# courtois-neuromod/phantom_vlb

Measured on AMD Instinct MI355X. Metric: clips/sec fine-tune VideoLLaMA2-7B+LoRA->2k-voxel head, 1/2/4/8 MI355X, higher is better.
Workload: dtype bf16; 1 GPU; configs[2]: VideoLLaMA2-7B + LoRA r=16 + 2k-voxel head, bf16; clips_per_gpu=3, global_batch=3, seq_len=2048, frames=12, num_target=2048, weights=random-init, comm=none

## Files before the change

### include/vlb.h

```cpp
#ifndef VLB_H
#define VLB_H

#include <stdint.h>

#ifdef __cplusplus
extern "C" {
#endif
#if defined(__GNUC__) || defined(__clang__)
#pragma GCC visibility push(default)
#endif

#define VLB_OK 0
#define VLB_ERR_INVALID (-1)
#define VLB_ERR_LAUNCH (-2)

#define VLB_ABI_VERSION 2

#define VLB_ACT_NONE 0
#define VLB_ACT_QUICK_GELU 1
#define VLB_ACT_GELU 2
#define VLB_ACT_SILU 3
#define VLB_ACT_SWIGLU_PAIR 4
#define VLB_ACT_SWIGLU_BWD 5

int vlb_abi_version(void);
const char* vlb_last_error(void);

int vlb_gemm_bf16(const void* A, int lda, const void* W, int ldw, void* C, int ldc, int M, int N, int K,
                  const void* bias, const void* residual, int ldr, int act, const void* A2, int lda2,
                  const void* W2, int ldw2, int K2, void* stream);

int vlb_gemm_bf16_ws(const void* A, int lda, const void* W, int ldw, void* C, int ldc, int M, int N, int K,
                     const void* bias, const void* residual, int ldr, int act, const void* A2, int lda2,
                     const void* W2, int ldw2, int K2, void* ws, int64_t ws_bytes, void* stream);
int vlb_gemm_swiglu_save(const void* A, int lda, const void* W_il, int ldw, void* H, int ldh, void* GU, int ldgu, int M, int N,
                         int K, const void* A2, int lda2, const void* W2_il, int ldw2, int K2, void* ws, int64_t ws_bytes,
                         void* stream);
int64_t vlb_gemm_workspace_bytes(void);
int vlb_gemm_plan(int M, int N, int K, int K2, int with_workspace);

int vlb_gemm_bf16_masked_pair(const void* A, int lda, const void* W, int ldw, void* C, int ldc, int M, int N, int K,
                              const void* A2, int lda2, const void* W2, int ldw2, float drop_p, uint32_t seed,
                              void* stream);

int vlb_gemm_bf16_masked_pair_ws(const void* A, int lda, const void* W, int ldw, void* C, int ldc, int M, int N, int K,
                                 const void* A2, int lda2, const void* W2, int ldw2, float drop_p, uint32_t seed,
                                 void* ws, int64_t ws_bytes, void* stream);

int vlb_gemm_masked_pair_swiglu_bwd(const void* dY, int lddy, const void* Wt, int ldw, const void* gu, int ldgu, void* dgu,
                                    int lddgu, int M, int ff, int K, const void* U, int ldu, const void* At, int ldat,
                                    float drop_p, uint32_t seed, void* ws, int64_t ws_bytes, void* stream);

int vlb_gemm_kernel_choice(int M, int N, int K, int K2);

int vlb_transpose_bf16(const void* in, void* out, int R, int C, void* stream);

int vlb_attention_fwd(const void* q, int ldq, const void* k, int ldk, const void* v, int ldv, void* out, int ldo,
                      float* lse, const uint8_t* key_mask, int B, int S, int Hq, int Hkv, int D, int causal,
                      float scale, const int* cu_rows, void* stream);

int vlb_attention_bwd(const void* q, int ldq, const void* k, int ldk, const void* v, int ldv, const void* out,
                      int ldo, const void* dout, int lddo, const float* lse, const uint8_t* key_mask, void* dq,
                      int lddq, void* dk, int lddk, void* dv, int lddv, float* delta, float* dq_acc, int B, int S,
                      int Hq, int Hkv, int D, int causal, float scale, const int* cu_rows, int total_rows,
                      void* stream);

int vlb_rmsnorm_fwd(const void* x, const void* w, void* y, int rows, int dim, float eps, void* stream);
int vlb_rmsnorm_bwd(const void* x, const void* w, const void* dy, const void* dx_in, void* dx, int rows, int dim,
                    float eps, void* stream);
int vlb_layernorm_fwd(const void* x, const void* w, const void* b, const void* residual, void* y, int rows, int dim,
                      float eps, int act, void* stream);

int vlb_rope_inplace(void* x, int ld, const float* cos_t, const float* sin_t, int rows, int S, int heads, int D,
                     int sign, const int* pos, void* stream);
int vlb_swiglu_fwd(const void* gu, void* out, int rows, int ff, void* stream);
int vlb_swiglu_bwd(const void* gu, const void* dout, void* dgu, int rows, int ff, void* stream);
int vlb_add_bf16(const void* a, const void* b, void* y, int64_t n, void* stream);

int vlb_patchify(const float* vision, void* patches, int N, int H, int W, int P, int Kpad, void* stream);
int vlb_vit_assemble(const void* patch_emb, const void* cls, const void* pos, void* tokens, int N, int G, int D,
                     void* stream);
int vlb_drop_cls(const void* tokens, void* out, int N, int G, int D, void* stream);

int vlb_dwconv3x3(const void* x, const void* w, void* y, int N, int H, int W, int C, void* stream);
int vlb_se_pool(const void* x, void* pooled, int N, int HW, int C, void* stream);
int vlb_se_scale(const void* x, const void* gate, void* y, int N, int HW, int C, void* stream);
int vlb_im2col3d_k2s2p1(const void* x, void* cols, int B, int T, int H, int W, int C, void* stream);

int vlb_splice_embed(const int64_t* ids, const void* embed_w, const void* video_tokens, void* embeds,
                     uint8_t* key_mask, int* err_flag, int B, int L, int Nv, int D, int64_t video_id, int vocab,
                     const int* cu_rows, int* row_pos, void* stream);
int vlb_weight_mask(const int64_t* padvals, const double* vis_w, const double* lang_w, float* wmask, int B, int F,
                    int Lw, int tokens_per_frame, int S, int round_bf16, void* stream);

int vlb_head_partial_rows(int S);
int64_t vlb_head_ws_floats(int B, int S, int E, int V);
int vlb_head_fwd(const void* hidden, const float* wmask, const void* ln1_w, const void* ln1_b, const void* ln2_w,
                 const void* ln2_b, const void* ridge_w, const void* ridge_b, const float* y, const float* keep_scale,
                 float* ws, float* stats, float* pooled_raw, float* sumw, float* zhat, float* ln2_rstd, void* z,
                 float* pred, float* loss_terms, int B, int S, int E, int V, float eps, float l2_lambda, const int* cu_rows,
                 void* stream);
int vlb_head_bwd(const void* hidden, const float* wmask, const void* ln1_w, const void* ln2_w, const void* ridge_w,
                 const float* y, const float* keep_scale, const float* stats, const float* pooled_raw,
                 const float* sumw, const float* zhat, const float* ln2_rstd, const void* z, const float* pred,
                 float* d_ridge_w, float* d_ridge_b, float* d_ln2_w, float* d_ln2_b, float* d_ln1_w, float* d_ln1_b,
                 float* ws, float* dz_ws, float* dpooled_ws, void* dhidden, int B, int S, int E, int V, float eps,
                 float l2_lambda, float loss_scale, float l2_scale, const int* cu_rows, int total_rows, void* stream);

int vlb_feature_cache_store(const float* pooled_raw, const float* sumw, const int32_t* rows, float* cache_pooled,
                            float* cache_sumw, int B, int E, int n_rows, void* stream);
int vlb_head_fwd_cached(const float* cache_pooled, const float* cache_sumw, const int32_t* rows, const void* ln1_w,
                        const void* ln1_b, const void* ln2_w, const void* ln2_b, const void* ridge_w, const void* ridge_b,
                        const float* y, const float* keep_scale, float* ws, float* pooled_raw, float* sumw, float* zhat,
                        float* ln2_rstd, void* z, float* pred, float* loss_terms, int B, int E, int V, int n_rows, float eps,
                        float l2_lambda, void* stream);
int vlb_head_bwd_cached(const void* ln1_w, const void* ln2_w, const void* ridge_w, const float* y, const float* keep_scale,
                        const float* pooled_raw, const float* sumw, const float* zhat, const float* ln2_rstd, const void* z,
                        const float* pred, float* d_ridge_w, float* d_ridge_b, float* d_ln2_w, float* d_ln2_b, float* d_ln1_w,
                        float* d_ln1_b, float* ws, float* dz_ws, float* dpooled_ws, int B, int E, int V, float eps,
                        float l2_lambda, float loss_scale, float l2_scale, void* stream);

int vlb_lora_down(const void* x, int ldx, const void* A, void* t, int ldt, int M, int K, int R, float scale,
                  float drop_p, const uint32_t* seeds_host, void* stream);
int vlb_lora_dx_masked(const void* u, int ldu, const void* At, int ldat, void* dx, int lddx, int M, int K, int R, float drop_p,
                       const uint32_t* seeds_host, void* stream);
int64_t vlb_wgrad_u_ws_floats(int M, int K);
int vlb_wgrad_skinny_u(const void* G, int ldg, const void* X, int ldx, float* dW, float* ws, int M, int K, float alpha,
                       float beta, const void* Bt, float u_scale, void* u, int ldu, float* u_ws, void* stream);
int vlb_wgrad_skinny_u_multi(const void* G, int ldg, const void* X, int ldx, int M, int nproj, const int* cols, float* const* dW,
                             const void* const* Bt, float* ws, float alpha, float beta, float u_scale, void* u, int ldu,
                             float* u_ws, void* stream);
int vlb_transpose16_scatter(const void* jobs, int n_jobs, void* stream);
int vlb_wgrad_splits(int M);
int vlb_wgrad_skinny(const void* G, int ldg, const void* X, int ldx, float* dW, float* ws, int M, int N, int K,
                     float alpha, float beta, float drop_p, const uint32_t* seeds_host, void* stream);

int vlb_sumsq_ws_floats(void);
int vlb_grad_sumsq(const float* g, int64_t n, float* sumsq, float* ws, void* stream);
int vlb_adamw_step(float* master, void* param_bf16, const float* grad, float* m, float* v, int64_t n, float lr,
                   float beta1, float beta2, float eps, float weight_decay, int step, const float* sumsq,
                   float max_norm, void* stream);
int vlb_grad_accum(float* acc, const float* g, int64_t n, int first, float* sumsq, float* ws, void* stream);
int vlb_grad_accum_bf16(float* acc, const void* g_bf16, int64_t n, int first, float* sumsq, float* ws, void* stream);

int vlb_transpose_pad(const void* in, int ld_in, void* out, int ld_out, int R, int C, int Rpad, void* stream);
int64_t vlb_norm_bwd_ws_floats(int rows, int dim);
int64_t vlb_colsum_ws_floats(int rows, int dim);
int vlb_rmsnorm_bwd_dw(const void* x, const void* dy, void* dw_bf16, float* ws, int rows, int dim, float eps, void* stream);
// ... 65 lines not shown
```

### phantom_vlb_amd/_lib.py

```python
from __future__ import annotations

import ctypes
import os
from ctypes import c_char_p, c_double, c_float, c_int, c_int64, c_void_p

import torch

_HERE = os.path.dirname(os.path.abspath(__file__))
LIB_PATH = os.environ.get("VLB_LIB") or os.path.join(_HERE, "libvlb.so")
IS_PRODUCT_LIB = os.path.abspath(LIB_PATH) == os.path.join(_HERE, "libvlb.so")

P, I, F, L = c_void_p, c_int, c_float, c_int64

SIGNATURES = {
    "vlb_abi_version": [],
    "vlb_last_error": [],
    "vlb_gemm_bf16": [P, I, P, I, P, I, I, I, I, P, P, I, I, P, I, P, I, I, P],
    "vlb_gemm_bf16_ws": [P, I, P, I, P, I, I, I, I, P, P, I, I, P, I, P, I, I, P, L, P],
    "vlb_gemm_swiglu_save": [P, I, P, I, P, I, P, I, I, I, I, P, I, P, I, I, P, L, P],
    "vlb_gemm_workspace_bytes": [],
    "vlb_gemm_plan": [I, I, I, I, I],
    "vlb_gemm_kernel_choice": [I, I, I, I],
    "vlb_transpose_bf16": [P, P, I, I, P],
    "vlb_attention_fwd": [P, I, P, I, P, I, P, I, P, P, I, I, I, I, I, I, F, P, P],
    "vlb_attention_bwd": [P, I, P, I, P, I, P, I, P, I, P, P, P, I, P, I, P, I, P, P, I, I, I, I, I, I, F, P, I, P],
    "vlb_rmsnorm_fwd": [P, P, P, I, I, F, P],
    "vlb_rmsnorm_bwd": [P, P, P, P, P, I, I, F, P],
    "vlb_layernorm_fwd": [P, P, P, P, P, I, I, F, I, P],
    "vlb_rope_inplace": [P, I, P, P, I, I, I, I, I, P, P],
    "vlb_swiglu_fwd": [P, P, I, I, P],
    "vlb_swiglu_bwd": [P, P, P, I, I, P],
    "vlb_add_bf16": [P, P, P, L, P],
    "vlb_patchify": [P, P, I, I, I, I, I, P],
    "vlb_vit_assemble": [P, P, P, P, I, I, I, P],
    "vlb_drop_cls": [P, P, I, I, I, P],
    "vlb_dwconv3x3": [P, P, P, I, I, I, I, P],
    "vlb_se_pool": [P, P, I, I, I, P],
    "vlb_se_scale": [P, P, P, I, I, I, P],
    "vlb_im2col3d_k2s2p1": [P, P, I, I, I, I, I, P],
    "vlb_splice_embed": [P, P, P, P, P, P, I, I, I, I, L, I, P, P, P],
    "vlb_weight_mask": [P, P, P, P, I, I, I, I, I, I, P],
    "vlb_head_partial_rows": [I],
    "vlb_head_ws_floats": [I, I, I, I],
    "vlb_head_fwd": [P] * 19 + [I, I, I, I, F, F, P, P],
    "vlb_head_bwd": [P] * 24 + [I, I, I, I, F, F, F, F, P, I, P],
    "vlb_feature_cache_store": [P] * 5 + [I, I, I, P],
    "vlb_head_fwd_cached": [P] * 19 + [I, I, I, I, F, F, P],
    "vlb_head_bwd_cached": [P] * 20 + [I, I, I, F, F, F, F, P],
    "vlb_gemm_bf16_masked_pair": [P, I, P, I, P, I, I, I, I, P, I, P, I, F, ctypes.c_uint32, P],
    "vlb_gemm_masked_pair_swiglu_bwd": [P, I, P, I, P, I, P, I, I, I, I, P, I, P, I, F, ctypes.c_uint32, P, L, P],
    "vlb_gemm_bf16_masked_pair_ws": [P, I, P, I, P, I, I, I, I, P, I, P, I, F, ctypes.c_uint32, P, L, P],
    "vlb_wgrad_u_ws_floats": [I, I],
    "vlb_wgrad_skinny_u": [P, I, P, I, P, P, I, I, F, F, P, F, P, I, P, P],
    "vlb_wgrad_skinny_u_multi": [P, I, P, I, I, I, P, P, P, P, F, F, F, P, I, P, P],
    "vlb_transpose16_scatter": [P, I, P],
    "vlb_wgrad_splits": [I],
    "vlb_wgrad_skinny": [P, I, P, I, P, P, I, I, I, F, F, F, P, P],
    "vlb_lora_down": [P, I, P, P, I, I, I, I, F, F, P, P],
    "vlb_lora_dx_masked": [P, I, P, I, P, I, I, I, I, F, P, P],
    "vlb_sumsq_ws_floats": [],
    "vlb_grad_sumsq": [P, L, P, P, P],
    "vlb_adamw_step": [P, P, P, P, P, L, F, F, F, F, F, I, P, F, P],
    "vlb_grad_accum": [P, P, L, I, P, P, P],
    "vlb_grad_accum_bf16": [P, P, L, I, P, P, P],
    "vlb_dropout_keep_scale": [P, L, F, ctypes.c_uint32, P],
    "vlb_transpose_pad": [P, I, P, I, I, I, I, P],
    "vlb_norm_bwd_ws_floats": [I, I],
    "vlb_colsum_ws_floats": [I, I],
    "vlb_rmsnorm_bwd_dw": [P, P, P, P, I, I, F, P],
    "vlb_rmsnorm_bwd_full_ws_floats": [I, I],
    "vlb_rmsnorm_bwd_full": [P, P, P, P, P, P, P, I, I, F, P],
    "vlb_layernorm_bwd": [P, P, P, P, P, P, P, P, P, P, I, I, F, I, P],
    "vlb_act_fwd": [P, P, L, I, P],
    "vlb_act_bwd": [P, P, P, L, I, P],
    "vlb_colsum": [P, I, P, P, I, I, P],
    "vlb_embed_grad": [P, I, P, P, P, I, P, I, P],
    "vlb_grad_sumsq_bf16": [P, L, P, P, P],
    "vlb_adamw_step_g16": [P, P, P, P, P, L, F, F, F, F, F, I, P, F, P],
    "vlb_dwconv3x3_bwd_w_ws_floats": [I, I, I],
    "vlb_dwconv3x3_bwd_w": [P, P, P, P, I, I, I, I, P],
    "vlb_se_bwd_gate": [P, P, P, P, I, I, I, P],
    "vlb_se_bwd_x": [P, P, P, P, I, I, I, P],
    "vlb_col2im3d_k2s2p1": [P, P, I, I, I, I, I, P],
    "vlb_quantize_mxfp8": [P, I, P, I, P, I, I, I, P],
    "vlb_transpose_quantize_mxfp8": [P, I, P, I, P, I, I, I, I, P],
    "vlb_quantize_dual_mxfp8": [P, I, P, I, P, I, P, I, P, I, I, I, I, P],
    "vlb_rmsnorm_fwd_mxfp8": [P, P, P, P, I, P, I, I, I, F, P],
    "vlb_swiglu_fwd_mxfp8": [P, P, P, I, P, I, I, I, P],
    "vlb_gemm_mxfp8": [P, I, P, I, P, I, P, I, P, I, I, I, I, P, I, P],
    "vlb_comm_unique_id": [P],
    "vlb_comm_init": [I, I, P, ctypes.POINTER(c_void_p)],
    "vlb_comm_destroy": [P],
    "vlb_comm_loopback_stage_bytes": [I],
    "vlb_comm_init_loopback": [I, P, L, ctypes.POINTER(c_void_p)],
    "vlb_comm_rank": [P],
    "vlb_comm_world": [P],
    "vlb_allgather_direct": [P, P, P, L, P],
    "vlb_reducescatter_stage_floats": [L, I],
    "vlb_reducescatter_direct": [P, P, P, L, P, P],
    "vlb_reducescatter_direct_bf16": [P, P, P, L, P, P],
    "vlb_reduce_slices": [P, P, L, I, I, P],
    "vlb_profile_marker": [P],
    "vlb_hrf_pool_ws_floats": [I, I],
    "vlb_hrf_pool": [P, I, P, P, P, I, I, I, P],
    "vlb_ridge_ws_floats": [I],
    "vlb_ridge_fwd": [P, P, P, P, P, P, I, I, I, F, P],
    "vlb_allreduce_scalar": [P, P, I, P],
    "vlb_cast_f32_to_bf16": [P, P, L, P],
# ... 36 lines not shown
```

### phantom_vlb_amd/csrc/attention.hip

```cpp
#include "common.hpp"

namespace {

constexpr int KV = 64;
constexpr int QW = 32;
constexpr int NW = 4;
constexpr int QB = QW * NW;
constexpr float NEG = -1e30f;

__device__ __forceinline__ void glds16(const void* g, void* l) {
  __builtin_amdgcn_global_load_lds((const void __attribute__((address_space(1)))*)g,
                                   (void __attribute__((address_space(3)))*)l, 16, 0, 0);
}

typedef short s16x4 __attribute__((ext_vector_type(4)));

__device__ __forceinline__ s16x4 tr_read_asm(const char* lds_ptr) {
  s16x4 v;
  const unsigned a = (unsigned)(uintptr_t)(const char __attribute__((address_space(3)))*)lds_ptr;
  asm volatile("ds_read_b64_tr_b16 %0, %1" : "=v"(v) : "v"(a));
  return v;
}
__device__ __forceinline__ void lds_wait_all() {
  asm volatile("s_waitcnt lgkmcnt(0)" ::: "memory");
// ... 182 lines not shown
          const int roff = (32 * s + 16 * s2) * ROWB;
#pragma unroll
          for (int dt = 0; dt < DT; ++dt) {
            const s16x4 lo = __builtin_amdgcn_ds_read_tr16_b64_v4i16(
                (s16x4 __attribute__((address_space(3)))*)(vb + v_rd[dt] + roff));
            const s16x4 hi = __builtin_amdgcn_ds_read_tr16_b64_v4i16(
                (s16x4 __attribute__((address_space(3)))*)(vb + v_rd[dt] + roff + 8 * ROWB));
            ot[dt] = __builtin_amdgcn_mfma_f32_32x32x16_bf16(join8(lo, hi), pf, ot[dt], 0, 0, 0);
          }
        }
    }
    asm volatile("s_waitcnt vmcnt(0)" ::: "memory");
    __syncthreads();
  }

  const float l_tot = l_run + __shfl_xor(l_run, 32, 64);
  const float inv = l_tot > 0.f ? 1.f / l_tot : 0.f;
  const int qrow = q0 + ql;
  if (qrow < Sb) {
    bf16* op = p.o + (row0 + qrow) * p.ldo + hq * D;
#pragma unroll
    for (int dt = 0; dt < DT; ++dt)
#pragma unroll
      for (int g = 0; g < 4; ++g) {
        bf16x4 o;
#pragma unroll
        for (int e = 0; e < 4; ++e) o[e] = (bf16)(ot[dt][4 * g + e] * inv);
        *reinterpret_cast<bf16x4*>(op + 32 * dt + 8 * g + 4 * h) = o;
      }
    if (p.lse && h == 0)
      p.lse[((int64_t)b * p.Hq + hq) * p.S + qrow] = l_tot > 0.f ? m_run * p.scale + logf(l_tot) : -INFINITY;
  }
}

template <int D, bool CAUSAL>
int launch_fwd(const AttnArgs& a, hipStream_t s) {
  constexpr int LDS = 2 * 2 * KV * D * 2;
  static const hipError_t attr = hipFuncSetAttribute(reinterpret_cast<const void*>(&attn_fwd_kernel<D, CAUSAL>),
                                                     hipFuncAttributeMaxDynamicSharedMemorySize, LDS);
  if (attr != hipSuccess) { vlb_set_error("attention: LDS reservation failed: %s", hipGetErrorString(attr)); return VLB_ERR_LAUNCH; }
  dim3 grid(((a.S + QB - 1) / QB) * a.Hq * a.B);
  hipLaunchKernelGGL((attn_fwd_kernel<D, CAUSAL>), grid, dim3(256), LDS, s, a);
  VLB_LAUNCH_CHECK();
  return VLB_OK;
}
}

extern "C" int vlb_attention_fwd(const void* q, int ldq, const void* k, int ldk, const void* v, int ldv, void* out,
                                 int ldo, float* lse, const uint8_t* key_mask, int B, int S, int Hq, int Hkv, int D,
                                 int causal, float scale, const int* cu_rows, void* stream) {
  VLB_REQUIRE(q && k && v && out, "attention_fwd: null operand");
  VLB_REQUIRE(D == 64 || D == 128, "attention_fwd: head dim %d not in {64,128}", D);
  VLB_REQUIRE(B > 0 && S > 0 && Hq > 0 && Hkv > 0 && Hq % Hkv == 0, "attention_fwd: bad shape B=%d S=%d Hq=%d Hkv=%d", B, S, Hq, Hkv);
  VLB_REQUIRE(ldq % 8 == 0 && ldk % 8 == 0 && ldv % 8 == 0 && ldo % 4 == 0, "attention_fwd: strides must keep 16-byte alignment");
  VLB_REQUIRE((((uintptr_t)q | (uintptr_t)k | (uintptr_t)v) % 16 == 0) && ((uintptr_t)out % 8 == 0), "attention_fwd: misaligned pointer");
  AttnArgs a{(const bf16*)q, (const bf16*)k, (const bf16*)v, (bf16*)out, lse, key_mask, cu_rows, ldq, ldk, ldv, ldo, B, S, Hq, Hkv, scale};
  hipStream_t s = as_stream(stream);
  if (D == 128) return causal ? launch_fwd<128, true>(a, s) : launch_fwd<128, false>(a, s);
  return causal ? launch_fwd<64, true>(a, s) : launch_fwd<64, false>(a, s);
}

namespace {

constexpr int BK_KEYS = 128;
constexpr int BQ = 32;

#ifdef VLB_TOOLS
int g_attn_ablate = 0;
#else
constexpr int g_attn_ablate = 0;
#endif
struct AttnBwdArgs {
  const bf16* q; const bf16* k; const bf16* v; const bf16* dout;
  const float* lse; const float* delta; const uint8_t* mask; const int* cu;
  bf16* dk; bf16* dv; float* dq_acc;
  int ldq, ldk, ldv, lddo, lddk, lddv;
  int B, S, Hq, Hkv;
  float scale;
  int ablate;
};

__device__ __forceinline__ int sw2(int r) { return ((r & 3) << 2) | ((r >> 2) & 3); }

__global__ __launch_bounds__(256) void attn_delta_kernel(const bf16* __restrict__ o, int ldo, const bf16* __restrict__ d_o,
                                                         int lddo, float* __restrict__ delta, int S, int Hq, int B,
                                                         const int* __restrict__ cu, int64_t total) {
  const int64_t gid = (int64_t)blockIdx.x * 16 + (threadIdx.x >> 4);
  const int c = threadIdx.x & 15;
  float s = 0.f;
  if (gid < total) {
    const int h = gid % Hq; const int64_t tok = gid / Hq;
    const bf16x8 a = *reinterpret_cast<const bf16x8*>(o + tok * ldo + h * 128 + c * 8);
    const bf16x8 b = *reinterpret_cast<const bf16x8*>(d_o + tok * lddo + h * 128 + c * 8);
#pragma unroll
    for (int i = 0; i < 8; ++i) s += (float)a[i] * (float)b[i];
  }
#pragma unroll
  for (int off = 8; off > 0; off >>= 1) s += __shfl_xor(s, off, 64);
  if (gid < total && c == 0) {
    const int h = gid % Hq; const int64_t tok = gid / Hq;
    int64_t b = tok / S; int sidx = tok % S;
    if (cu) {
      int bb = 0;
      while (bb + 1 < B && tok >= cu[bb + 1]) ++bb;
      b = bb; sidx = (int)(tok - cu[bb]);
    }
    delta[(b * Hq + h) * S + sidx] = s;
  }
}

template <bool CAUSAL>
__global__ __launch_bounds__(256, 2) void attn_bwd_dkdv_kernel(AttnBwdArgs p, bf16* __restrict__ part) {
  constexpr int D = 128, ROWB = 256;
  constexpr int V_OFF = 0;
  constexpr int QT_BYTES = BQ * ROWB;
  constexpr int Q_OFF = BK_KEYS * ROWB;
  constexpr int L_OFF = Q_OFF + 4 * QT_BYTES;
  extern __shared__ __attribute__((aligned(16))) char smem[];

  const int tid = threadIdx.x, lane = tid & 63;
  const int w4 = __builtin_amdgcn_readfirstlane(tid >> 6);
  const int per_kb = p.Hq * p.B;
  const int kb = blockIdx.x / per_kb, hq = xcd_head((blockIdx.x % per_kb) % p.Hq, p.Hq), b = (blockIdx.x % per_kb) / p.Hq;
  const int gsz = p.Hq / p.Hkv;
  const int hkv = hq / gsz;
  const int k0 = kb * BK_KEYS;
  const int Sb = p.cu ? p.cu[b + 1] - p.cu[b] : p.S;
  const int64_t row0 = p.cu ? p.cu[b] : (int64_t)b * p.S;
  if (k0 >= Sb) return;
  const int ql = lane & 31, h = lane >> 5;
  const int g1 = (lane >> 4) & 1, li = lane & 15, tq = li >> 2, tp = li & 3;
  const int sr = lane >> 4, sp = lane & 15;

  const int krow = w4 * 32 + ql;
  const int key = k0 + krow;
  bf16x8 kf[8];
  {
    const bf16* kp = p.k + (row0 + min(key, Sb - 1)) * p.ldk + hkv * D + 8 * h;
#pragma unroll
    for (int ks = 0; ks < 8; ++ks) kf[ks] = *reinterpret_cast<const bf16x8*>(kp + 16 * ks);
  }
  const bf16* vbase = p.v + row0 * p.ldv + hkv * D;
#pragma unroll
  for (int i = 0; i < 8; ++i) {
    const int piece = 4 * i + w4, r = piece * 4 + sr;
    glds16(vbase + (int64_t)min(k0 + r, Sb - 1) * p.ldv + (sp ^ sw2(r)) * 8, smem + V_OFF + piece * 1024);
  }
  const int nqb = (Sb + BQ - 1) / BQ;
  const int qb0 = CAUSAL ? (k0 / BQ) : 0;
  const int total = nqb - qb0;
  const bf16* qbase = p.q + row0 * p.ldq + hq * D;
  const bf16* dobase = p.dout + row0 * p.lddo + hq * D;
  const float* lsebase = p.lse + ((int64_t)b * p.Hq + hq) * p.S;
  const float* delbase = p.delta + ((int64_t)b * p.Hq + hq) * p.S;

  auto stage_q = [&](int buf, int item) {
    const int qb = qb0 + item;
    char* qt = smem + Q_OFF + buf * 2 * QT_BYTES;
#pragma unroll
    for (int i = 0; i < 2; ++i) {
      const int piece = 4 * i + w4, r = piece * 4 + sr;
      const int qr = min(qb * BQ + r, Sb - 1);
      glds16(qbase + (int64_t)qr * p.ldq + (sp ^ sw2(r)) * 8, qt + piece * 1024);
      glds16(dobase + (int64_t)qr * p.lddo + (sp ^ sw2(r)) * 8, qt + QT_BYTES + piece * 1024);
    }
    if (w4 == 0) {
      const int qr = min(qb * BQ + (lane & 31), Sb - 1);
      const float* src = (lane < 32 ? lsebase : delbase) + qr;
      __builtin_amdgcn_global_load_lds((const void __attribute__((address_space(1)))*)src,
                                       (void __attribute__((address_space(3)))*)(smem + L_OFF + buf * 256), 4, 0, 0);
    }
  };

  f32x16 dkt[4], dvt[4];
#pragma unroll
  for (int i = 0; i < 4; ++i)
#pragma unroll
    for (int r = 0; r < 16; ++r) { dkt[i][r] = 0.f; dvt[i][r] = 0.f; }
// ... 38 lines not shown
        pacc = __builtin_amdgcn_mfma_f32_32x32x16_bf16(dof, vf, pacc, 0, 0, 0);
      }
      bf16x8 pb[2], dsb[2];
#pragma unroll
      for (int g = 0; g < 4; ++g) {
        const f32x4 l4 = *reinterpret_cast<const f32x4*>(ls + 8 * g + 4 * h);
        const f32x4 d4 = *reinterpret_cast<const f32x4*>(ls + 32 + 8 * g + 4 * h);
#pragma unroll
        for (int e = 0; e < 4; ++e) {
          const int r = 4 * g + e;
          const int qrow = q0 + 8 * g + 4 * h + e;
          bool ok = key_ok && qrow < Sb;
          if (CAUSAL) ok = ok && (key <= qrow);
          const float pv = ok ? __builtin_amdgcn_exp2f(sacc[r] * c2 - l4[e] * 1.44269504088896341f) : 0.f;
          const float ds = pv * (pacc[r] - d4[e]) * p.scale;
          pb[r >> 3][r & 7] = (bf16)pv;
          dsb[r >> 3][r & 7] = (bf16)ds;
        }
      }
#pragma unroll
      for (int s = 0; s < 2; ++s) {
        s16x4 ra[4][2];
#pragma unroll
        for (int dt = 0; dt < 4; ++dt)
#pragma unroll
          for (int e = 0; e < 2; ++e) ra[dt][e] = tr_read_asm(dot + qt_rd[dt][e] + 16 * s * ROWB);
        lds_wait_all();
#pragma unroll
        for (int dt = 0; dt < 4; ++dt)
          dvt[dt] = __builtin_amdgcn_mfma_f32_32x32x16_bf16(join8(ra[dt][0], ra[dt][1]), pb[s], dvt[dt], 0, 0, 0);
#pragma unroll
        for (int dt = 0; dt < 4; ++dt)
#pragma unroll
          for (int e = 0; e < 2; ++e) ra[dt][e] = tr_read_asm(qt + qt_rd[dt][e] + 16 * s * ROWB);
        lds_wait_all();
#pragma unroll
        for (int dt = 0; dt < 4; ++dt)
          dkt[dt] = __builtin_amdgcn_mfma_f32_32x32x16_bf16(join8(ra[dt][0], ra[dt][1]), dsb[s], dkt[dt], 0, 0, 0);
      }
    }
    asm volatile("s_waitcnt vmcnt(0)" ::: "memory");
    asm volatile("s_waitcnt lgkmcnt(0)" ::: "memory");
    __builtin_amdgcn_s_barrier();
  }

  if (key < Sb) {
    bf16* dkp = gsz == 1 ? p.dk + (row0 + key) * p.lddk + hkv * D : part + ((row0 + key) * p.Hq + hq) * (2 * D);
    bf16* dvp = gsz == 1 ? p.dv + (row0 + key) * p.lddv + hkv * D : dkp + D;
#pragma unroll
    for (int dt = 0; dt < 4; ++dt)
#pragma unroll
      for (int g = 0; g < 4; ++g) {
        bf16x4 a, c;
#pragma unroll
        for (int e = 0; e < 4; ++e) { a[e] = (bf16)dkt[dt][4 * g + e]; c[e] = (bf16)dvt[dt][4 * g + e]; }
        *reinterpret_cast<bf16x4*>(dkp + 32 * dt + 8 * g + 4 * h) = a;
        *reinterpret_cast<bf16x4*>(dvp + 32 * dt + 8 * g + 4 * h) = c;
      }
  }
}

__global__ __launch_bounds__(256) void attn_dkdv_reduce_kernel(const bf16* __restrict__ part, bf16* __restrict__ dk, int lddk,
                                                               bf16* __restrict__ dv, int lddv, int Hq, int Hkv, int64_t total) {
  const int64_t i = blockIdx.x * (int64_t)blockDim.x + threadIdx.x;
  if (i >= total) return;
  const int c = i & 15, which = (i >> 4) & 1;
  const int hkv = (int)((i >> 5) % Hkv);
  const int64_t row = (i >> 5) / Hkv;
  const int gsz = Hq / Hkv;
  float acc[8] = {0.f, 0.f, 0.f, 0.f, 0.f, 0.f, 0.f, 0.f};
  const bf16* src = part + (row * Hq + (int64_t)hkv * gsz) * 256 + which * 128 + c * 8;
  for (int j = 0; j < gsz; ++j) {
    const bf16x8 v = *reinterpret_cast<const bf16x8*>(src + (int64_t)j * 256);
#pragma unroll
    for (int e = 0; e < 8; ++e) acc[e] += (float)v[e];
  }
  bf16x8 o;
#pragma unroll
  for (int e = 0; e < 8; ++e) o[e] = (bf16)acc[e];
  bf16* dst = which ? dv + row * lddv : dk + row * lddk;
  *reinterpret_cast<bf16x8*>(dst + hkv * 128 + c * 8) = o;
}

struct AttnDqArgs {
  const bf16* q; const bf16* k; const bf16* v; const bf16* dout;
  const float* lse; const float* delta; const uint8_t* mask; const int* cu;
  bf16* dq;
  int ldq, ldk, ldv, lddo, lddq;
  int B, S, Hq, Hkv;
  float scale;
};

template <bool CAUSAL>
__global__ __launch_bounds__(256, 2) void attn_bwd_dq_kernel(AttnDqArgs p) {
  constexpr int D = 128, ROWB = 256, TILE = KV * ROWB, KS = 8, DT = 4;
  extern __shared__ __attribute__((aligned(16))) char smem[];

  const int tid = threadIdx.x, lane = tid & 63;
  const int wave = __builtin_amdgcn_readfirstlane(tid >> 6);
  const int nqb = (p.S + QB - 1) / QB;
  const int per_qb = p.Hq * p.B, slot = blockIdx.x / per_qb;
  const int qb = CAUSAL ? (nqb - 1 - slot) : slot;
  const int hq = xcd_head((blockIdx.x % per_qb) % p.Hq, p.Hq), b = (blockIdx.x % per_qb) / p.Hq;
  const int hkv = hq / (p.Hq / p.Hkv);
  const int Sb = p.cu ? p.cu[b + 1] - p.cu[b] : p.S;
  const int64_t row0 = p.cu ? p.cu[b] : (int64_t)b * p.S;
  if (qb * QB >= Sb) return;
  const int q0 = qb * QB + wave * QW;
  const int ql = lane & 31, h = lane >> 5;
  const int qrow = q0 + ql;
  const int qr = min(qrow, Sb - 1);

  bf16x8 qf[KS], dof[KS];
  {
    const bf16* qp = p.q + (row0 + qr) * p.ldq + hq * D + 8 * h;
    const bf16* dp = p.dout + (row0 + qr) * p.lddo + hq * D + 8 * h;
#pragma unroll
    for (int ks = 0; ks < KS; ++ks) {
      qf[ks] = *reinterpret_cast<const bf16x8*>(qp + 16 * ks);
      dof[ks] = *reinterpret_cast<const bf16x8*>(dp + 16 * ks);
    }
  }
  const float lse_q = p.lse[((int64_t)b * p.Hq + hq) * p.S + qr];
  const float delta_q = p.delta[((int64_t)b * p.Hq + hq) * p.S + qr];
  const float c2 = p.scale * 1.44269504088896341f;
  const float lse2 = (lse_q > -1e37f) ? lse_q * 1.44269504088896341f : 1e37f;

  f32x16 dqt[DT];
#pragma unroll
  for (int i = 0; i < DT; ++i)
#pragma unroll
    for (int r = 0; r < 16; ++r) dqt[i][r] = 0.f;

  const int q_hi = min(qb * QB + QB, Sb) - 1;
  const int ntiles = CAUSAL ? (q_hi / KV + 1) : (Sb + KV - 1) / KV;
  const bf16* kbase = p.k + row0 * p.ldk + hkv * D;
  const bf16* vbase = p.v + row0 * p.ldv + hkv * D;

  const int sr = lane >> 4, sp = lane & 15;
  auto stage = [&](int buf, int t) {
    char* kb = smem + buf * 2 * TILE; char* vb = kb + TILE;
#pragma unroll
    for (int i = 0; i < 4; ++i) {
      const int r = (4 * i + wave) * 4 + sr;
      const int key = min(t * KV + r, Sb - 1);
      glds16(kbase + (int64_t)key * p.ldk + (sp ^ sw2(r)) * 8, kb + (4 * i + wave) * 1024);
      glds16(vbase + (int64_t)key * p.ldv + (sp ^ sw2(r)) * 8, vb + (4 * i + wave) * 1024);
    }
  };
  stage(0, 0);
  asm volatile("s_waitcnt vmcnt(0)" ::: "memory");
  __syncthreads();

  const int g1 = (lane >> 4) & 1, li = lane & 15, tq = li >> 2, tp = li & 3;
  int row_rd[KS];
#pragma unroll
  for (int ks = 0; ks < KS; ++ks) row_rd[ks] = ql * ROWB + (((2 * ks + h) ^ sw2(ql)) << 4);
  int tr_rd[DT][2];
#pragma unroll
  for (int dt = 0; dt < DT; ++dt)
#pragma unroll
    for (int e = 0; e < 2; ++e) {
      const int r = 4 * h + tq + 8 * e;
      tr_rd[dt][e] = r * ROWB + (((4 * dt + 2 * g1 + (tp >> 1)) ^ sw2(r)) << 4) + (tp & 1) * 8;
    }

  for (int t = 0; t < ntiles; ++t) {
    const int cur = t & 1;
    if (t + 1 < ntiles) stage(cur ^ 1, t + 1);
    const char* kb = smem + cur * 2 * TILE; const char* vb = kb + TILE;
    const int key0 = t * KV;
    const bool active = !CAUSAL || (key0 <= q0 + QW - 1);
    if (active) {
      f32x16 st[2], dp[2];
#pragma unroll
      for (int s = 0; s < 2; ++s)
#pragma unroll
        for (int r = 0; r < 16; ++r) { st[s][r] = 0.f; dp[s][r] = 0.f; }
#pragma unroll
      for (int ks = 0; ks < KS; ++ks) {
#pragma unroll
        for (int s = 0; s < 2; ++s) {
          const bf16x8 kf = *reinterpret_cast<const bf16x8*>(kb + row_rd[ks] + 32 * s * ROWB);
          st[s] = __builtin_amdgcn_mfma_f32_32x32x16_bf16(kf, qf[ks], st[s], 0, 0, 0);
          const bf16x8 vf = *reinterpret_cast<const bf16x8*>(vb + row_rd[ks] + 32 * s * ROWB);
          dp[s] = __builtin_amdgcn_mfma_f32_32x32x16_bf16(vf, dof[ks], dp[s], 0, 0, 0);
        }
      }
      unsigned long long kvalid;
      {
        const int key = key0 + lane;
        bool ok = key < Sb;
        if (ok && p.mask) ok = p.mask[row0 + key] != 0;
        kvalid = __ballot(ok);
      }
      const bool diag = CAUSAL && (key0 + KV - 1 > q0);
      const bool partial = diag || (kvalid != ~0ull);
      if (partial) {
        const unsigned lo = (unsigned)(kvalid >> (4 * h)), hi = (unsigned)(kvalid >> (32 + 4 * h));
#pragma unroll
        for (int s = 0; s < 2; ++s) {
          const unsigned word = s ? hi : lo;
#pragma unroll
          for (int r = 0; r < 16; ++r) {
            const int kb2 = (r & 3) + 8 * (r >> 2);
            bool ok = (word >> kb2) & 1u;
            if (CAUSAL) ok = ok && (key0 + 32 * s + 4 * h + kb2 <= qrow);
            st[s][r] = ok ? st[s][r] : NEG;
          }
        }
        asm volatile("" ::: "memory");
      }
#pragma unroll
      for (int s = 0; s < 2; ++s)
#pragma unroll
        for (int r = 0; r < 16; ++r) {
          const float pv = __builtin_amdgcn_exp2f(st[s][r] * c2 - lse2);
          st[s][r] = pv * (dp[s][r] - delta_q) * p.scale;
        }
#pragma unroll
      for (int s = 0; s < 2; ++s)
#pragma unroll
        for (int s2 = 0; s2 < 2; ++s2) {
          bf16x8 df;
#pragma unroll
          for (int j = 0; j < 8; ++j) df[j] = (bf16)st[s][8 * s2 + j];
          const int roff = (32 * s + 16 * s2) * ROWB;
#pragma unroll
          for (int dt = 0; dt < DT; ++dt) {
            const s16x4 lo = __builtin_amdgcn_ds_read_tr16_b64_v4i16(
                (s16x4 __attribute__((address_space(3)))*)(kb + tr_rd[dt][0] + roff));
            const s16x4 hi = __builtin_amdgcn_ds_read_tr16_b64_v4i16(
                (s16x4 __attribute__((address_space(3)))*)(kb + tr_rd[dt][1] + roff));
            dqt[dt] = __builtin_amdgcn_mfma_f32_32x32x16_bf16(join8(lo, hi), df, dqt[dt], 0, 0, 0);
          }
        }
    }
    asm volatile("s_waitcnt vmcnt(0)" ::: "memory");
    __syncthreads();
  }

  if (qrow < Sb) {
    bf16* op = p.dq + (row0 + qrow) * p.lddq + hq * D;
#pragma unroll
    for (int dt = 0; dt < DT; ++dt)
#pragma unroll
      for (int g = 0; g < 4; ++g) {
        bf16x4 o;
#pragma unroll
        for (int e = 0; e < 4; ++e) o[e] = (bf16)dqt[dt][4 * g + e];
        *reinterpret_cast<bf16x4*>(op + 32 * dt + 8 * g + 4 * h) = o;
      }
  }
}

}

extern "C" int vlb_attention_bwd(const void* q, int ldq, const void* k, int ldk, const void* v, int ldv, const void* out,
                                 int ldo, const void* dout, int lddo, const float* lse, const uint8_t* key_mask, void* dq,
                                 int lddq, void* dk, int lddk, void* dv, int lddv, float* delta, float* dq_acc, int B,
                                 int S, int Hq, int Hkv, int D, int causal, float scale, const int* cu_rows, int total_rows,
                                 void* stream) {
  VLB_REQUIRE(q && k && v && out && dout && lse && dq && dk && dv && delta, "attention_bwd: null operand");
  VLB_REQUIRE(dq_acc || Hq == Hkv, "attention_bwd: the [rows, Hq, D] fp32-sized workspace is required");
  VLB_REQUIRE(D == 128, "attention_bwd: head dim %d unsupported (only 128: the decoder)", D);
  VLB_REQUIRE(B > 0 && S > 0 && Hq > 0 && Hkv > 0 && Hq % Hkv == 0, "attention_bwd: bad shape");
  VLB_REQUIRE(ldq % 8 == 0 && ldk % 8 == 0 && ldv % 8 == 0 && ldo % 8 == 0 && lddo % 8 == 0 && lddq % 8 == 0 &&
                  lddk % 4 == 0 && lddv % 4 == 0, "attention_bwd: strides must keep vector alignment");
  VLB_REQUIRE(((((uintptr_t)q | (uintptr_t)k | (uintptr_t)v | (uintptr_t)out | (uintptr_t)dout) % 16) == 0) &&
                  ((uintptr_t)dq % 8 == 0), "attention_bwd: misaligned pointer");
  hipStream_t st = as_stream(stream);
  const int64_t rows = cu_rows ? (int64_t)total_rows : (int64_t)B * S;
  VLB_REQUIRE(rows > 0 && rows <= (int64_t)B * S, "attention_bwd: total_rows=%d out of range", total_rows);
  const int64_t th = rows * Hq;
  hipLaunchKernelGGL(attn_delta_kernel, dim3((unsigned)((th + 15) / 16)), dim3(256), 0, st, (const bf16*)out, ldo,
                     (const bf16*)dout, lddo, delta, S, Hq, B, cu_rows, th);
  VLB_LAUNCH_CHECK();
  AttnBwdArgs a{(const bf16*)q, (const bf16*)k, (const bf16*)v, (const bf16*)dout, lse, delta, key_mask, cu_rows,
                (bf16*)dk, (bf16*)dv, dq_acc, ldq, ldk, ldv, lddo, lddk, lddv, B, S, Hq, Hkv, scale, g_attn_ablate};
  dim3 grid((S + BK_KEYS - 1) / BK_KEYS, Hkv, B);
  {
    const int gsz = Hq / Hkv;
    VLB_REQUIRE(gsz == 1 || dq_acc, "attention_bwd: the workspace (fp32 [rows, Hq, D]) is required for grouped-query heads");
    VLB_REQUIRE(lddk % 8 == 0 && lddv % 8 == 0 && (((uintptr_t)dk | (uintptr_t)dv) % 16) == 0, "attention_bwd: dk/dv rows must be 16-byte aligned");
    constexpr int LDS_KV = BK_KEYS * 256 + 4 * BQ * 256 + 512;
    static const hipError_t k1 = hipFuncSetAttribute(reinterpret_cast<const void*>(&attn_bwd_dkdv_kernel<true>), hipFuncAttributeMaxDynamicSharedMemorySize, LDS_KV);
    static const hipError_t k2 = hipFuncSetAttribute(reinterpret_cast<const void*>(&attn_bwd_dkdv_kernel<false>), hipFuncAttributeMaxDynamicSharedMemorySize, LDS_KV);
    if (k1 != hipSuccess || k2 != hipSuccess) { vlb_set_error("attention_bwd: LDS reservation failed (dk/dv)"); return VLB_ERR_LAUNCH; }
    bf16* part = reinterpret_cast<bf16*>(dq_acc);
    dim3 gridh(grid.x * Hq * B);
    if (causal) hipLaunchKernelGGL(attn_bwd_dkdv_kernel<true>, gridh, dim3(256), LDS_KV, st, a, part);
    else hipLaunchKernelGGL(attn_bwd_dkdv_kernel<false>, gridh, dim3(256), LDS_KV, st, a, part);
    VLB_LAUNCH_CHECK();
    if (gsz > 1) {
      const int64_t tot = rows * Hkv * 32;
      hipLaunchKernelGGL(attn_dkdv_reduce_kernel, dim3((unsigned)((tot + 255) / 256)), dim3(256), 0, st, part, (bf16*)dk, lddk,
                         (bf16*)dv, lddv, Hq, Hkv, tot);
      VLB_LAUNCH_CHECK();
    }
  }
  AttnDqArgs d{(const bf16*)q, (const bf16*)k, (const bf16*)v, (const bf16*)dout, lse, delta, key_mask, cu_rows,
               (bf16*)dq, ldq, ldk, ldv, lddo, lddq, B, S, Hq, Hkv, scale};
  constexpr int LDS_DQ = 2 * 2 * KV * 256;
  static const hipError_t q1 = hipFuncSetAttribute(reinterpret_cast<const void*>(&attn_bwd_dq_kernel<true>), hipFuncAttributeMaxDynamicSharedMemorySize, LDS_DQ);
  static const hipError_t q2 = hipFuncSetAttribute(reinterpret_cast<const void*>(&attn_bwd_dq_kernel<false>), hipFuncAttributeMaxDynamicSharedMemorySize, LDS_DQ);
  if (q1 != hipSuccess || q2 != hipSuccess) { vlb_set_error("attention_bwd: LDS reservation failed (dq)"); return VLB_ERR_LAUNCH; }
  dim3 gq(((S + QB - 1) / QB) * Hq * B);
  if (causal) hipLaunchKernelGGL(attn_bwd_dq_kernel<true>, gq, dim3(256), LDS_DQ, st, d);
  else hipLaunchKernelGGL(attn_bwd_dq_kernel<false>, gq, dim3(256), LDS_DQ, st, d);
  VLB_LAUNCH_CHECK();
  return VLB_OK;
}

#ifdef VLB_TOOLS
extern "C" void vlb_attn_set_ablation(int bits) { g_attn_ablate = bits & 3; }
#endif
```

### phantom_vlb_amd/csrc/common.hpp

```cpp
#pragma once
#include <hip/hip_runtime.h>
#include <stdint.h>
#include <stdio.h>
#include <string.h>

#include "../../include/vlb.h"

typedef __bf16 bf16;
typedef __bf16 bf16x2 __attribute__((ext_vector_type(2)));
typedef __bf16 bf16x4 __attribute__((ext_vector_type(4)));
typedef __bf16 bf16x8 __attribute__((ext_vector_type(8)));
typedef float f32x2 __attribute__((ext_vector_type(2)));
typedef float f32x4 __attribute__((ext_vector_type(4)));
typedef float f32x16 __attribute__((ext_vector_type(16)));
typedef unsigned int u32x2 __attribute__((ext_vector_type(2)));
typedef unsigned int u32x4 __attribute__((ext_vector_type(4)));

#define VLB_WAVE 64

void vlb_set_error(const char* fmt, ...);

#define VLB_REQUIRE(cond, ...)                 \
  do {                                         \
    if (!(cond)) {                             \
      vlb_set_error(__VA_ARGS__);              \
      return VLB_ERR_INVALID;                  \
    }                                          \
  } while (0)

#define VLB_LAUNCH_CHECK()                                                   \
  do {                                                                       \
    hipError_t e__ = hipGetLastError();                                      \
    if (e__ != hipSuccess) {                                                 \
      vlb_set_error("%s:%d launch failed: %s", __FILE__, __LINE__,           \
                    hipGetErrorString(e__));                                 \
      return VLB_ERR_LAUNCH;                                                 \
    }                                                                        \
  } while (0)

static inline hipStream_t as_stream(void* s) {
  (void)hipGetLastError();
  return reinterpret_cast<hipStream_t>(s);
}

__device__ __forceinline__ float bf2f(bf16 x) { return (float)x; }
__device__ __forceinline__ bf16 f2bf(float x) { return (bf16)x; }

__device__ __forceinline__ float wave_sum(float v) {
#pragma unroll
  for (int o = 32; o > 0; o >>= 1) v += __shfl_xor(v, o, 64);
  return v;
}
__device__ __forceinline__ float wave_max(float v) {
#pragma unroll
  for (int o = 32; o > 0; o >>= 1) v = fmaxf(v, __shfl_xor(v, o, 64));
  return v;
}

__device__ __forceinline__ float block_sum(float v, float* red) {
  v = wave_sum(v);
  const int w = threadIdx.x >> 6, nw = blockDim.x >> 6;
  __syncthreads();
  if ((threadIdx.x & 63) == 0) red[w] = v;
  __syncthreads();
  float t = 0.f;
  for (int i = 0; i < nw; ++i) t += red[i];
  return t;
}

__device__ __forceinline__ float sigmoid_f(float x) { return __builtin_amdgcn_rcpf(1.f + __expf(-x)); }
__device__ __forceinline__ float silu_f(float x) { return x * sigmoid_f(x); }
__device__ __forceinline__ float quick_gelu_f(float x) { return x * sigmoid_f(1.702f * x); }
__device__ __forceinline__ float gelu_erf_f(float x) { return 0.5f * x * (1.f + erff(x * 0.70710678118654752f)); }

__device__ __forceinline__ int mx_shared_exp(float amax) {
  int E = -127;
  if (amax > 0.f) {
    int e; const float f = frexpf(amax / 448.f, &e);
    E = (f == 0.5f) ? e - 1 : e;
    E = max(-127, min(127, E));
  }
  return E;
}
__device__ __forceinline__ uint32_t mx_pack4(float a, float b, float c, float d, float inv) {
  int pk = 0;
  pk = __builtin_amdgcn_cvt_pk_fp8_f32(a * inv, b * inv, pk, false);
  pk = __builtin_amdgcn_cvt_pk_fp8_f32(c * inv, d * inv, pk, true);
  return (uint32_t)pk;
}
__device__ __forceinline__ void mx_quantize_lane8(const float (&v)[8], uint8_t* qrow, uint8_t* srow, int c, int lane) {
  float amax = 0.f;
#pragma unroll
  for (int i = 0; i < 8; ++i) amax = fmaxf(amax, fabsf(v[i]));
  amax = fmaxf(amax, __shfl_xor(amax, 1, 64));
  amax = fmaxf(amax, __shfl_xor(amax, 2, 64));
  const int E = mx_shared_exp(amax);
  const float inv = exp2f((float)-E);
  typedef unsigned u32x2_ __attribute__((ext_vector_type(2)));
  *reinterpret_cast<u32x2_*>(qrow + c) = u32x2_{mx_pack4(v[0], v[1], v[2], v[3], inv), mx_pack4(v[4], v[5], v[6], v[7], inv)};
  if ((lane & 3) == 0) srow[c >> 5] = (uint8_t)(E + 127);
}
__device__ __forceinline__ void load_pair16(const bf16* row, int n, int fq, bf16x4& a, bf16x4& b) {
  typedef unsigned u32x2 __attribute__((ext_vector_type(2)));
  typedef unsigned u32x4 __attribute__((ext_vector_type(4)));
  const u32x4 l = *reinterpret_cast<const u32x4*>(row + n + ((fq & 1) ? 12 : 0));
  const auto r0 = __builtin_amdgcn_permlane16_swap(l[0], l[2], false, false);
  const auto r1 = __builtin_amdgcn_permlane16_swap(l[1], l[3], false, false);
  a = __builtin_bit_cast(bf16x4, u32x2{r0[0], r1[0]});
  b = __builtin_bit_cast(bf16x4, u32x2{r0[1], r1[1]});
}
__device__ __forceinline__ void store_pair16(bf16* row, int n, bf16x4 a, bf16x4 b, int fq) {
  typedef unsigned u32x2 __attribute__((ext_vector_type(2)));
  typedef unsigned u32x4 __attribute__((ext_vector_type(4)));
  u32x2 ua = __builtin_bit_cast(u32x2, a), ub = __builtin_bit_cast(u32x2, b);
  const auto r0 = __builtin_amdgcn_permlane16_swap(ua[0], ub[0], false, false);
  const auto r1 = __builtin_amdgcn_permlane16_swap(ua[1], ub[1], false, false);
  const u32x4 o = {r0[0], r1[0], r0[1], r1[1]};
  *reinterpret_cast<u32x4*>(row + n + ((fq & 1) ? 12 : 0)) = o;
}
```

### phantom_vlb_amd/csrc/gemm.hip

```cpp
#include <type_traits>

#include "common.hpp"

namespace {

constexpr int BK = 64;
constexpr int ROW_BYTES = BK * 2;

struct GemmArgs {
  const bf16* A;  const bf16* W;  bf16* C;
  const bf16* A2; const bf16* W2;
  const bf16* bias; const bf16* residual;
  int M, N, K, K2;
  int lda, ldw, ldc, ldr, lda2, ldw2;
  int act;
  int tiles_m, tiles_n;
  int tile0;
  int split_n;
  int grid;
  uint32_t drop_thresh, drop_key; float drop_scale;
  float* ws; int k_splits, tail_tiles;
  int order;
  bf16* aux; int ldaux;
  int reserved;
  int wide;
};

__device__ __forceinline__ void tile_coords(const GemmArgs& p, int pid, int sub, int BM, int BN, int& m0, int& n0) {
  int tm, tn;
  if (p.order & 4) {
    const int sbt = 16 * p.tiles_m;
    const int sb = pid / sbt, c0 = sb * 16;
    const int wd = min(p.tiles_n - c0, 16);
    int w = pid - sb * sbt;
    const int rg = w / (4 * wd);
    const int gsz = min(p.tiles_m - 4 * rg, 4);
    w -= rg * 4 * wd;
    const int h = w / (gsz * 8);
    const int cw = min(wd - 8 * h, 8);
    w -= h * gsz * 8;
    tm = 4 * rg + w / cw;
    tn = c0 + 8 * h + w % cw;
  } else if (p.order & 1) {
    constexpr int GROUP_N = 8;
    const int band = GROUP_N * p.tiles_m;
    const int cb = pid / band, c0 = cb * GROUP_N;
    const int csz = min(p.tiles_n - c0, GROUP_N);
    const int w = pid - cb * band;
    tm = w / csz;
    tn = c0 + w % csz;
  } else {
    constexpr int GROUP_M = 4;
    const int band = GROUP_M * p.tiles_n;
    const int g0 = (pid / band) * GROUP_M;
    const int gsz = min(p.tiles_m - g0, GROUP_M);
    tm = g0 + (pid % band) % gsz;
    tn = (pid % band) / gsz;
  }
  m0 = tm * BM;
  n0 = (tn * p.split_n + sub) * BN;
}

__device__ __forceinline__ int xcd_remap_pid(int order) {
  const int nblk = gridDim.x, pid = blockIdx.x;
  const int x = pid & 7, j = pid >> 3;
  int base = 0, n = nblk, jj = j;
  if (order & 2) {
    const int T = nblk >> 8, t = j >> 5;
    if (t < T) return (t << 8) + (x << 5) + (j & 31);
    base = T << 8; n = nblk - base; jj = j - (T << 5);
  }
  const int q = n >> 3, r = n & 7;
  return base + (x < r ? x * (q + 1) : r * (q + 1) + (x - r) * q) + jj;
}

__device__ __forceinline__ int map_tile(const GemmArgs& p, int BM, int BN, int& m0, int& n0) {
  int pid = xcd_remap_pid(p.order);
  int sub = 0, ks = 0;
  if (p.split_n > 1) { sub = pid % p.split_n; pid /= p.split_n; }
  if (p.k_splits > 1) { ks = pid / p.tail_tiles; pid -= ks * p.tail_tiles; }
  tile_coords(p, pid + p.tile0, sub, BM, BN, m0, n0);
  return ks;
}

__device__ __forceinline__ float apply_act(float x, int act) {
  switch (act) {
    case VLB_ACT_QUICK_GELU: return quick_gelu_f(x);
    case VLB_ACT_GELU: return gelu_erf_f(x);
    case VLB_ACT_SILU: return silu_f(x);
    default: return x;
  }
}

__device__ __forceinline__ void store_swiglu4(const GemmArgs& p, const f32x4& g, const f32x4& u, int m, int n) {
  bf16x4 o;
#pragma unroll
  for (int e = 0; e < 4; ++e) o[e] = (bf16)(silu_f(g[e]) * u[e]);
  *reinterpret_cast<bf16x4*>(p.C + (int64_t)m * p.ldc + n) = o;
  if (p.aux) {
    bf16x4 gb, ub;
#pragma unroll
    for (int e = 0; e < 4; ++e) { gb[e] = (bf16)g[e]; ub[e] = (bf16)u[e]; }
    bf16* ap = p.aux + (int64_t)m * p.ldaux + n;
    *reinterpret_cast<bf16x4*>(ap) = gb;
    *reinterpret_cast<bf16x4*>(ap + (p.N >> 1)) = ub;
  }
}

// ... 492 lines not shown
        if (g >= 1 && (g * 4) % NT == 0 && g * 4 / NT - 1 <= MT - 2) af[g * 4 / NT - 1] = frag(sn, a_off[0], g * 4 / NT - 1);
        if (g == LAST_A) a7[0] = frag(sn, a_off[0], MT - 1);
      }
#pragma unroll
      for (int q = 0; q < 4; ++q) {
        const int t = g * 4 + q, i = t / NT, j = t % NT;
        mfma_tied(acc[i][j], wf[1][j], i == MT - 1 ? a7[1] : af[i]);
      }
      W4_FENCE();
    }
    __builtin_amdgcn_s_waitcnt(0xc07f);
    asm volatile("s_nop 15" ::: "memory");
    W4_FENCE();
  };
  using T_ = std::true_type; using F_ = std::false_type;
  int kt = 0;
  if constexpr (MASKED) {
    const bool later_range = SPLITK && ksplit != 0;
    const uint32_t m_thresh = later_range ? 0u : p.drop_thresh;
    const float m_scale = later_range ? 1.f : p.drop_scale;
    tile(0, T_{}, T_{});
    kt = 1;
    asm volatile("s_nop 15\n\ts_nop 15" ::: "memory");
#pragma unroll
    for (int i = 0; i < MT; ++i)
#pragma unroll
      for (int j = 0; j < NT; j += 4)
        asm volatile("" : "+a"(acc[i][j]), "+a"(acc[i][j + 1]), "+a"(acc[i][j + 2]), "+a"(acc[i][j + 3]));
    const int frm = lane & 15, fqm = lane >> 4;
    const uint32_t halfN = (uint32_t)(p.N >> 1);
#pragma unroll
    for (int i = 0; i < MT; ++i) {
      const uint32_t rb = (uint32_t)(m0 + wm * TM + i * 16 + frm) * halfN;
#pragma unroll
      for (int j = 0; j < NT; ++j) {
        const uint32_t pair0 = (uint32_t)(n0 + wn * TN + j * 16 + fqm * 4) >> 1;
        f32x4 v = acc[i][j];
#pragma unroll
        for (int q = 0; q < 2; ++q) {
          uint32_t h = (rb + pair0 + q) ^ p.drop_key;
          h ^= h >> 16; h *= 0x7feb352dU; h ^= h >> 15; h *= 0x846ca68bU; h ^= h >> 16;
          v[2 * q] = (h & 0xffffu) >= m_thresh ? v[2 * q] * m_scale : 0.f;
          v[2 * q + 1] = (h >> 16) >= m_thresh ? v[2 * q + 1] * m_scale : 0.f;
        }
        acc[i][j] = v;
        asm volatile("" : "+a"(acc[i][j]));
        W4_FENCE();
      }
    }
    asm volatile("s_nop 7" ::: "memory");
  }
  for (; kt + 2 < nk; ++kt) tile(kt, T_{}, T_{});
  if (kt + 1 < nk) { tile(kt, T_{}, F_{}); ++kt; }
  tile(kt, F_{}, F_{});
  asm volatile("s_nop 15\n\ts_nop 15" ::: "memory");
#pragma unroll
  for (int i = 0; i < MT; ++i)
#pragma unroll
    for (int j = 0; j < NT; j += 4)
      asm volatile("" : "+a"(acc[i][j]), "+a"(acc[i][j + 1]), "+a"(acc[i][j + 2]), "+a"(acc[i][j + 3]));
#undef W4_FENCE
#undef W4_BARRIER

  if constexpr (SPLITK) {
    float* wt = p.ws + ((int64_t)xcd_remap_pid(p.order) * 4 + wave) * (MT * NT * 256);
#pragma unroll
    for (int i = 0; i < MT; ++i)
#pragma unroll
      for (int j = 0; j < NT; ++j)
        *reinterpret_cast<f32x4*>(wt + ((i * NT + j) * 64 + lane) * 4) = acc[i][j];
    return;
  }
  if (p.act == VLB_ACT_SWIGLU_PAIR) {
#pragma unroll
    for (int i = 0; i < MT; ++i) {
      const int m = m0 + wm * TM + i * 16 + fr;
      if (m >= p.M) continue;
#pragma unroll
      for (int j = 0; j < NT; j += 4)
        store_swiglu8(p, acc[i][j], acc[i][j + 1], acc[i][j + 2], acc[i][j + 3], m, (n0 + wn * TN) / 2 + (j / 2) * 16 + fq * 4, fq);
    }
    return;
  }
#define W4_EPILOGUE(KIND)                                                                                              \
  _Pragma("unroll") for (int i = 0; i < MT; ++i) {                                                                      \
    const int m = m0 + wm * TM + i * 16 + fr;                                                                           \
    if (m >= p.M) continue;                                                                                             \
    _Pragma("unroll") for (int j = 0; j < NT; j += 2)                                                                   \
      w4_store_frag2<KIND>(p, acc[i][j], acc[i][j + 1], m, n0 + wn * TN + j * 16 + fq * 4, fq);                         \
  }
  const int kind = w4_epilogue_kind(p);
  if (kind == EPI_PLAIN) { W4_EPILOGUE(EPI_PLAIN) return; }
  if (kind == EPI_RESIDUAL) { W4_EPILOGUE(EPI_RESIDUAL) return; }
  if (kind == EPI_SWIGLU_BWD) { W4_EPILOGUE(EPI_SWIGLU_BWD) return; }
#define W4_EPILOGUE_ACT(ACT) W4_EPILOGUE(EPI_GENERIC + ACT)
  VLB_DISPATCH_ACT(p.act, W4_EPILOGUE_ACT);
#undef W4_EPILOGUE_ACT
#undef W4_EPILOGUE
}

template <int MT, int NT>
__global__ __launch_bounds__(256) void gemm_splitk_reduce_kernel(GemmArgs p) {
  constexpr int TM = 16 * MT, TN = 16 * NT, BM = 2 * TM, BN = 2 * TN;
  const int tl = blockIdx.x / MT, i = blockIdx.x % MT;
  int m0, n0;
  tile_coords(p, p.tile0 + tl, 0, BM, BN, m0, n0);
  const int lane = threadIdx.x & 63, wave = threadIdx.x >> 6;
  const int wm = wave >> 1, wn = wave & 1, fr = lane & 15, fq = lane >> 4;
  f32x4 v[NT];
#pragma unroll
  for (int j = 0; j < NT; ++j) v[j] = f32x4{0.f, 0.f, 0.f, 0.f};
  for (int s = 0; s < p.k_splits; ++s) {
    const float* wt = p.ws + ((int64_t)(s * p.tail_tiles + tl) * 4 + wave) * (MT * NT * 256);
#pragma unroll
    for (int j = 0; j < NT; ++j) v[j] += *reinterpret_cast<const f32x4*>(wt + ((i * NT + j) * 64 + lane) * 4);
  }
  const int m = m0 + wm * TM + i * 16 + fr;
  if (m >= p.M) return;
  if (p.act == VLB_ACT_SWIGLU_PAIR) {
#pragma unroll
    for (int j = 0; j < NT; j += 4) store_swiglu8(p, v[j], v[j + 1], v[j + 2], v[j + 3], m, (n0 + wn * TN) / 2 + (j / 2) * 16 + fq * 4, fq);
    return;
  }
  const int kind = w4_epilogue_kind(p);
#define W4_REDUCE_EPILOGUE(KIND) \
  _Pragma("unroll") for (int j = 0; j < NT; j += 2) w4_store_frag2<KIND>(p, v[j], v[j + 1], m, n0 + wn * TN + j * 16 + fq * 4, fq);
  if (kind == EPI_PLAIN) { W4_REDUCE_EPILOGUE(EPI_PLAIN) return; }
  if (kind == EPI_RESIDUAL) { W4_REDUCE_EPILOGUE(EPI_RESIDUAL) return; }
  if (kind == EPI_SWIGLU_BWD) { W4_REDUCE_EPILOGUE(EPI_SWIGLU_BWD) return; }
#define W4_REDUCE_EPILOGUE_ACT(ACT) W4_REDUCE_EPILOGUE(EPI_GENERIC + ACT)
  VLB_DISPATCH_ACT(p.act, W4_REDUCE_EPILOGUE_ACT);
#undef W4_REDUCE_EPILOGUE_ACT
#undef W4_REDUCE_EPILOGUE
}

template <int NT, int ABL, int MT = 8, bool MASKED = false, bool SPLITK = false>
int launch_w4(GemmArgs& a, hipStream_t s) {
  constexpr int LDS = 2 * (32 * MT + 32 * NT) * ROW_BYTES;
  static const hipError_t attr = hipFuncSetAttribute(reinterpret_cast<const void*>(&gemm_w4_kernel<NT, ABL, MT, MASKED, SPLITK>),
                                       hipFuncAttributeMaxDynamicSharedMemorySize, LDS);
  if (attr != hipSuccess) {
    vlb_set_error("gemm: cannot reserve %d bytes of LDS: %s", LDS, hipGetErrorString(attr));
    return VLB_ERR_LAUNCH;
  }
  hipLaunchKernelGGL((gemm_w4_kernel<NT, ABL, MT, MASKED, SPLITK>), dim3(a.grid), dim3(256), LDS, s, a);
  VLB_LAUNCH_CHECK();
  return VLB_OK;
}

template <int MT, bool MASKED = false>
int launch_w4_splitk(GemmArgs& a, hipStream_t s) {
  a.split_n = 1;
  a.grid = a.k_splits * a.tail_tiles;
  int rc = launch_w4<8, 0, MT, MASKED, true>(a, s);
  if (rc != VLB_OK) return rc;
  hipLaunchKernelGGL((gemm_splitk_reduce_kernel<MT, 8>), dim3(a.tail_tiles * MT), dim3(256), 0, s, a);
  VLB_LAUNCH_CHECK();
  return VLB_OK;
}

#ifdef VLB_TOOLS
#define VLB_TUNABLE
#else
#define VLB_TUNABLE constexpr
#endif
VLB_TUNABLE int g_variant = 3;
// ... 63 lines not shown
  return launch_pp<BM, BN, WM, WN, (BM + BN) / 64, 0, 0, 0>(a, s, LDS);
#else
  if constexpr (BM == 256 && BN == 256) {
    if (!fits32 && (g_variant == 2 || (g_variant >= 0x20 && g_variant < 0x30))) return launch_pp<BM, BN, WM, WN, (BM + BN) / 64, 0, 0, 0>(a, s, LDS);
    if (g_variant == 2) return launch_w4<8, 0>(a, s);
    if (g_variant == 3 || g_variant == 4 || g_variant == 5 || g_variant == 6) {
      if (fits32 && a.K + a.K2 >= 4096) return launch_w4<8, 0>(a, s);
      return launch_pp<BM, BN, WM, WN, (BM + BN) / 64, 0, 0, 0>(a, s, LDS);
    }
    if (g_variant == 0x21) return launch_w4<8, 1>(a, s);
    if (g_variant == 0x22) return launch_w4<8, 2>(a, s);
    if (g_variant == 0x24) return launch_w4<8, 4>(a, s);
    if (g_variant == 0x27) return launch_w4<8, 7>(a, s);
    if (g_variant == 0x28) return launch_w4<8, 8>(a, s);
    if (g_variant == 0x41) return launch_w4<8, 16>(a, s);
    if (g_variant == 0x42) return launch_w4<8, 32>(a, s);
    if (g_variant == 0x43) return launch_w4<8, 48>(a, s);
  } else {
    if constexpr (BM == 256 && BN == 128) {
      if ((g_variant == 2 || g_variant == 3 || g_variant == 5 || g_variant == 6) && fits32 && a.K + a.K2 >= 4096) return launch_w4<4, 0>(a, s);
    }
    if (g_variant == 2 || g_variant == 3 || g_variant == 4 || g_variant == 5 || g_variant == 6 || g_variant >= 0x20) return launch_pp<BM, BN, WM, WN, (BM + BN) / 64, 0, 0, 0>(a, s, LDS);
  }
  if (g_variant == 1) return launch_pp<BM, BN, WM, WN, (BM + BN) / 64, 0, 0, 0>(a, s, LDS);
  constexpr int T = (BM + BN) / 64;
  if constexpr (BM == 256 && BN == 256) {
    if (g_variant == 0x11) return launch_pp<BM, BN, WM, WN, T, 0, 0, 0, 1>(a, s, LDS);
    if (g_variant == 0x12) return launch_pp<BM, BN, WM, WN, T, 0, 0, 0, 2>(a, s, LDS);
    if (g_variant == 0x14) return launch_pp<BM, BN, WM, WN, T, 0, 0, 0, 4>(a, s, LDS);
    if (g_variant == 0x13) return launch_pp<BM, BN, WM, WN, T, 0, 0, 0, 3>(a, s, LDS);
    if (g_variant == 0x17) return launch_pp<BM, BN, WM, WN, T, 0, 0, 0, 7>(a, s, LDS);
    if (g_variant == 0x16) return launch_pp<BM, BN, WM, WN, T, 0, 0, 0, 6>(a, s, LDS);
  }
  if (g_variant >= 0x10) return launch_pp<BM, BN, WM, WN, T, 0, 0, 0>(a, s, LDS);
  vlb_set_error("gemm: unknown kernel variant %d", g_variant);
  return VLB_ERR_INVALID;
#endif
}

__global__ void transpose_kernel(const bf16* __restrict__ in, bf16* __restrict__ out, int R, int C) {
  __shared__ bf16 t[32][33];
  const int c0 = blockIdx.x * 32, r0 = blockIdx.y * 32;
  for (int i = threadIdx.y; i < 32; i += blockDim.y) {
    const int r = r0 + i, c = c0 + threadIdx.x;
    if (r < R && c < C) t[i][threadIdx.x] = in[(int64_t)r * C + c];
  }
  __syncthreads();
  for (int i = threadIdx.y; i < 32; i += blockDim.y) {
    const int c = c0 + i, r = r0 + threadIdx.x;
    if (r < R && c < C) out[(int64_t)c * R + r] = t[threadIdx.x][i];
  }
}

}

extern "C" int vlb_gemm_kernel_choice(int M, int N, int K, int K2) {
  if (K % BK != 0 || K2 % BK != 0 || K == 0 || M < 128) return 0;
  const int cus = 256;
  if (N % 256 == 0) {
    const int t256 = ((M + 255) / 256) * (N / 256);
    if (t256 < cus / 2) return 2;
    return 1;
  }
  if (N % 128 == 0) return 2;
  return 0;
}

extern "C" int vlb_gemm_plan(int M, int N, int K, int K2, int with_workspace) {
  if (N % 256 != 0 || K + K2 < 4096) return 0;
  TailPlan p256, p192;
  const bool use192 = plan_rows(M, N, K + K2, (with_workspace & 1) != 0, p256, p192, !(with_workspace & 2));
  const TailPlan& t = use192 ? p192 : p256;
  return (use192 ? 192 : 256) * 1000 + t.mode * 100 + t.splits;
}

extern "C" int64_t vlb_gemm_workspace_bytes(void) { return 256ll * 256 * 256 * 4; }

extern "C" int vlb_gemm_bf16(const void* A, int lda, const void* W, int ldw, void* C, int ldc, int M, int N, int K,
                             const void* bias, const void* residual, int ldr, int act, const void* A2, int lda2,
                             const void* W2, int ldw2, int K2, void* stream) {
  return vlb_gemm_bf16_ws(A, lda, W, ldw, C, ldc, M, N, K, bias, residual, ldr, act, A2, lda2, W2, ldw2, K2, nullptr, 0, stream);
}

static int gemm_impl(const void* A, int lda, const void* W, int ldw, void* C, int ldc, int M, int N, int K,
                     const void* bias, const void* residual, int ldr, int act, const void* A2, int lda2,
                     const void* W2, int ldw2, int K2, void* ws, int64_t ws_bytes, void* stream, void* aux, int ldaux);

extern "C" int vlb_gemm_bf16_ws(const void* A, int lda, const void* W, int ldw, void* C, int ldc, int M, int N, int K,
                                const void* bias, const void* residual, int ldr, int act, const void* A2, int lda2,
                                const void* W2, int ldw2, int K2, void* ws, int64_t ws_bytes, void* stream) {
  return gemm_impl(A, lda, W, ldw, C, ldc, M, N, K, bias, residual, ldr, act, A2, lda2, W2, ldw2, K2, ws, ws_bytes, stream, nullptr, 0);
}

extern "C" int vlb_gemm_swiglu_save(const void* A, int lda, const void* W_il, int ldw, void* H, int ldh, void* GU, int ldgu, int M, int N,
                                    int K, const void* A2, int lda2, const void* W2_il, int ldw2, int K2, void* ws, int64_t ws_bytes,
                                    void* stream) {
  VLB_REQUIRE(GU && ldgu >= N && ldgu % 4 == 0 && N % 8 == 0 && ((uintptr_t)GU % 8) == 0,
              "gemm_swiglu_save: [gate | up] rows must hold N columns, 8-byte aligned (N=%d ldgu=%d)", N, ldgu);
  return gemm_impl(A, lda, W_il, ldw, H, ldh, M, N, K, nullptr, nullptr, 0, VLB_ACT_SWIGLU_PAIR, A2, lda2, W2_il, ldw2, K2, ws, ws_bytes,
                   stream, GU, ldgu);
}

static int gemm_impl(const void* A, int lda, const void* W, int ldw, void* C, int ldc, int M, int N, int K,
                     const void* bias, const void* residual, int ldr, int act, const void* A2, int lda2,
                     const void* W2, int ldw2, int K2, void* ws, int64_t ws_bytes, void* stream, void* aux, int ldaux) {
  VLB_REQUIRE(A && W && C, "gemm: null operand");
  VLB_REQUIRE(!ws || ((uintptr_t)ws % 16) == 0, "gemm: workspace must be 16-byte aligned");
  const bool ws_ok = ws && ws_bytes >= vlb_gemm_workspace_bytes();
  VLB_REQUIRE(M > 0 && N > 0 && K > 0, "gemm: bad shape M=%d N=%d K=%d", M, N, K);
  VLB_REQUIRE(K % 8 == 0 && lda % 8 == 0 && ldw % 8 == 0, "gemm: K/lda/ldw must be multiples of 8 (K=%d lda=%d ldw=%d)", K, lda, ldw);
  VLB_REQUIRE(lda >= K && ldw >= K && (ldc >= N || (act == VLB_ACT_SWIGLU_PAIR && ldc >= N / 2)), "gemm: leading dimension smaller than row");
  if (K2 > 0) {
    VLB_REQUIRE(A2 && W2, "gemm: K2>0 needs A2 and W2");
    VLB_REQUIRE(K2 % 8 == 0 && lda2 % 8 == 0 && ldw2 % 8 == 0 && lda2 >= K2 && ldw2 >= K2, "gemm: bad second operand pair");
  } else {
    A2 = nullptr; W2 = nullptr; K2 = 0;
  }
  if (residual) VLB_REQUIRE(ldr >= N, "gemm: ldr < N");
  if (act == VLB_ACT_SWIGLU_PAIR) {
    VLB_REQUIRE(N % 32 == 0 && !bias && !residual && ldc >= N / 2, "gemm: SWIGLU_PAIR needs N %% 32 == 0, no bias/residual, ldc >= N/2");
  }
  GemmArgs a;
  a.A = (const bf16*)A; a.W = (const bf16*)W; a.C = (bf16*)C;
  a.A2 = (const bf16*)A2; a.W2 = (const bf16*)W2;
  a.bias = (const bf16*)bias; a.residual = (const bf16*)residual;
  a.M = M; a.N = N; a.K = K; a.K2 = K2;
  a.lda = lda; a.ldw = ldw; a.ldc = ldc; a.ldr = ldr; a.lda2 = lda2; a.ldw2 = ldw2;
  a.act = act; a.tiles_m = 0; a.tiles_n = 0; a.tile0 = 0; a.split_n = 1; a.grid = 0; a.drop_thresh = 0; a.drop_key = 0; a.drop_scale = 1.f;
  a.ws = nullptr; a.k_splits = 0; a.tail_tiles = 0; a.order = pick_order(M, N, K); a.aux = (bf16*)aux; a.ldaux = ldaux;
  a.wide = ((uintptr_t)C % 16) == 0 && ldc % 8 == 0 && (!aux || (((uintptr_t)aux % 16) == 0 && ldaux % 8 == 0 && (N / 2) % 8 == 0));
  hipStream_t s = as_stream(stream);
  const bool vec_ok = (ldc % 4 == 0) && (!residual || ldr % 4 == 0) && (!aux || (ldaux % 4 == 0 && (N / 2) % 4 == 0)) &&
                      (((uintptr_t)C | (uintptr_t)residual | (uintptr_t)bias | (uintptr_t)aux) % 8 == 0) &&
                      (((uintptr_t)A | (uintptr_t)W | (uintptr_t)A2 | (uintptr_t)W2) % 16 == 0);
  int choice = vec_ok ? vlb_gemm_kernel_choice(M, N, K, K2) : 0;
  if (choice != 0 && g_force_tile == 1 && N % 256 == 0) choice = 1;
  if (choice != 0 && g_force_tile == 2 && N % 128 == 0) choice = 2;
  if (choice == 1) {
    const int cus = 256, tn = N / 256, tm = (M + 255) / 256;
    const int tiles = tm * tn, rem = tiles % cus;
    {
      const bool fits32 = a.wide && (int64_t)M * lda < (1ll << 31) && (int64_t)N * ldw < (1ll << 31) &&
                          (int64_t)M * lda2 < (1ll << 31) && (int64_t)N * ldw2 < (1ll << 31);
#ifdef VLB_TOOLS
      const int abl192 = (g_variant >= 0x30 && g_variant < 0x40) ? (g_variant & 0xf) : 0;
      const bool w4 = (g_variant == 3 || g_variant == 5 || g_variant == 6 || (g_variant >= 0x30 && g_variant < 0x40)) && fits32 && K + K2 >= 4096;
#else
      const bool w4 = (g_variant == 3 || g_variant == 5) && fits32 && K + K2 >= 4096;
#endif
      const int tm192 = (M + 191) / 192, tiles192 = tm192 * tn;
      TailPlan p256, p192;
      bool use192 = plan_rows(M, N, K + K2, ws_ok && w4, p256, p192);
#ifdef VLB_TOOLS
      if (g_variant == 6) use192 = false;
#endif
      if (w4 && g_force_tile == 0 && tiles > cus && (g_variant == 5 || (g_variant >= 0x30 && g_variant < 0x40) || use192)) {
        GemmArgs hi = a;
        hi.tiles_m = tm192; hi.tiles_n = tn; hi.tile0 = 0; hi.split_n = 1;
        const int rem192 = tiles192 % cus;
        hi.grid = p192.mode ? tiles192 - rem192 : tiles192;
#ifdef VLB_TOOLS
        if (abl192 == 1) return launch_w4<8, 1, 6>(hi, s);
        if (abl192 == 2) return launch_w4<8, 2, 6>(hi, s);
        if (abl192 == 4) return launch_w4<8, 4, 6>(hi, s);
        if (abl192 == 8) return launch_w4<8, 8, 6>(hi, s);
        if (abl192 == 7) return launch_w4<8, 7, 6>(hi, s);
        if (abl192 == 9) return launch_w4<8, 16, 6>(hi, s);
        if (abl192 == 10) return launch_w4<8, 32, 6>(hi, s);
        if (abl192 == 11) return launch_w4<8, 48, 6>(hi, s);
#endif
        int rc = launch_w4<8, 0, 6>(hi, s);
        if (rc != VLB_OK || !p192.mode) return rc;
        GemmArgs lo = hi;
        lo.tile0 = tiles192 - rem192;
        if (p192.mode == 2) {
          lo.ws = (float*)ws; lo.k_splits = p192.splits; lo.tail_tiles = rem192;
          return launch_w4_splitk<6>(lo, s);
        }
        lo.split_n = 2; lo.grid = 2 * rem192;
        return launch_w4<4, 0, 6>(lo, s);
      }
      if (w4 && g_force_tile == 0 && p256.mode == 2) {
        GemmArgs hi = a;
        hi.tiles_m = tm; hi.tiles_n = tn; hi.tile0 = 0; hi.split_n = 1; hi.grid = tiles - rem;
        int rc = launch_w4<8, 0, 8>(hi, s);
        if (rc != VLB_OK) return rc;
        GemmArgs lo = hi;
        lo.tile0 = tiles - rem; lo.ws = (float*)ws; lo.k_splits = p256.splits; lo.tail_tiles = rem;
        return launch_w4_splitk<8>(lo, s);
      }
    }
    if (g_tail_split && tiles > cus && rem != 0 && rem <= cus * 5 / 8) {
      GemmArgs hi = a, lo = a;
      hi.tiles_m = lo.tiles_m = tm;
      hi.tiles_n = lo.tiles_n = tn;
      hi.tile0 = 0; hi.split_n = 1; hi.grid = tiles - rem;
      lo.tile0 = tiles - rem; lo.split_n = 2; lo.grid = 2 * rem;
      int rc = launch_tile<256, 256, 2, 4>(hi, s);
      if (rc != VLB_OK) return rc;
      return launch_tile<256, 128, 4, 2>(lo, s);
    }
    return launch_tile<256, 256, 2, 4>(a, s);
  }
  if (choice == 2) return launch_tile<256, 128, 4, 2>(a, s);
  dim3 grid((N + 63) / 64, (M + 63) / 64);
  hipLaunchKernelGGL(gemm_generic_kernel, grid, dim3(256), 0, s, a);
  VLB_LAUNCH_CHECK();
  return VLB_OK;
}

namespace {
inline uint32_t lowbias32_h(uint32_t x) {
  x ^= x >> 16; x *= 0x7feb352dU; x ^= x >> 15; x *= 0x846ca68bU; x ^= x >> 16;
  return x;
}
}

extern "C" int vlb_gemm_bf16_masked_pair(const void* A, int lda, const void* W, int ldw, void* C, int ldc, int M, int N, int K,
                                         const void* A2, int lda2, const void* W2, int ldw2, float drop_p, uint32_t seed,
                                         void* stream) {
  return vlb_gemm_bf16_masked_pair_ws(A, lda, W, ldw, C, ldc, M, N, K, A2, lda2, W2, ldw2, drop_p, seed, nullptr, 0, stream);
}

static int masked_pair_impl(const void* A, int lda, const void* W, int ldw, void* C, int ldc, int M, int N, int K,
                            const void* A2, int lda2, const void* W2, int ldw2, float drop_p, uint32_t seed,
                            void* ws, int64_t ws_bytes, void* stream, int act, const void* residual, int ldr);

extern "C" int vlb_gemm_bf16_masked_pair_ws(const void* A, int lda, const void* W, int ldw, void* C, int ldc, int M, int N, int K,
                                            const void* A2, int lda2, const void* W2, int ldw2, float drop_p, uint32_t seed,
                                            void* ws, int64_t ws_bytes, void* stream) {
  return masked_pair_impl(A, lda, W, ldw, C, ldc, M, N, K, A2, lda2, W2, ldw2, drop_p, seed, ws, ws_bytes, stream, VLB_ACT_NONE, nullptr, 0);
}

extern "C" int vlb_gemm_masked_pair_swiglu_bwd(const void* dY, int lddy, const void* Wt, int ldw, const void* gu, int ldgu, void* dgu,
                                               int lddgu, int M, int ff, int K, const void* U, int ldu, const void* At, int ldat,
                                               float drop_p, uint32_t seed, void* ws, int64_t ws_bytes, void* stream) {
  VLB_REQUIRE(gu && dgu, "gemm_masked_pair_swiglu_bwd: null activation pointers");
  VLB_REQUIRE(ldgu >= 2 * ff && lddgu >= 2 * ff && ldgu % 8 == 0 && lddgu % 8 == 0 && ff % 8 == 0 && ((uintptr_t)gu % 16) == 0 && ((uintptr_t)dgu % 16) == 0,
              "gemm_masked_pair_swiglu_bwd: [gate|up] rows must hold 2*ff columns; gu and d gu rows 16-byte aligned (ff=%d ldgu=%d lddgu=%d)", ff, ldgu, lddgu);
  return masked_pair_impl(dY, lddy, Wt, ldw, dgu, lddgu, M, ff, K, U, ldu, At, ldat, drop_p, seed, ws, ws_bytes, stream,
                          VLB_ACT_SWIGLU_BWD, gu, ldgu);
}

static int masked_pair_impl(const void* A, int lda, const void* W, int ldw, void* C, int ldc, int M, int N, int K,
                            const void* A2, int lda2, const void* W2, int ldw2, float drop_p, uint32_t seed,
                            void* ws, int64_t ws_bytes, void* stream, int act, const void* residual, int ldr) {
  VLB_REQUIRE(!ws || ((uintptr_t)ws % 16) == 0, "gemm_masked_pair: workspace must be 16-byte aligned");
  const bool ws_ok = ws && ws_bytes >= vlb_gemm_workspace_bytes();
  VLB_REQUIRE(A && W && C && A2 && W2, "gemm_masked_pair: null operand");
  VLB_REQUIRE(M > 0 && N % 256 == 0 && K >= 128 && K % 64 == 0, "gemm_masked_pair: needs N %% 256 == 0, K %% 64 == 0, K >= 128 (N=%d K=%d)", N, K);
  VLB_REQUIRE(lda % 8 == 0 && ldw % 8 == 0 && lda2 % 8 == 0 && ldw2 % 8 == 0 && lda >= K && ldw >= K && lda2 >= 64 && ldw2 >= 64 &&
                  ldc % 4 == 0 && ldc >= N, "gemm_masked_pair: bad leading dimensions");
  VLB_REQUIRE((((uintptr_t)A | (uintptr_t)W | (uintptr_t)A2 | (uintptr_t)W2 | (uintptr_t)C) % 16) == 0 && ldc % 8 == 0,
              "gemm_masked_pair: operands and C rows must be 16-byte aligned");
  VLB_REQUIRE(drop_p > 0.f && drop_p < 1.f, "gemm_masked_pair: drop_p must be in (0,1) - use vlb_gemm_bf16 when p == 0");
  VLB_REQUIRE((int64_t)M * lda < (1ll << 31) && (int64_t)N * ldw < (1ll << 31) && (int64_t)M * lda2 < (1ll << 31) &&
                  (int64_t)N * ldw2 < (1ll << 31) && (int64_t)M * (N >> 1) < (1ll << 32),
              "gemm_masked_pair: operand too large for 32-bit offsets / the 32-bit dropout counter");
  GemmArgs a;
  a.A = (const bf16*)A; a.W = (const bf16*)W; a.C = (bf16*)C;
  a.A2 = (const bf16*)A2; a.W2 = (const bf16*)W2;
  a.bias = nullptr; a.residual = (const bf16*)residual;
  a.M = M; a.N = N; a.K = K; a.K2 = 64;
  a.lda = lda; a.ldw = ldw; a.ldc = ldc; a.ldr = ldr; a.lda2 = lda2; a.ldw2 = ldw2;
  a.act = act; a.tiles_m = 0; a.tiles_n = 0; a.tile0 = 0; a.split_n = 1; a.grid = 0;
  a.ws = nullptr; a.k_splits = 0; a.tail_tiles = 0; a.order = pick_order(M, N, K); a.aux = nullptr; a.ldaux = 0;
  a.wide = 1;
  uint32_t t = (uint32_t)(drop_p * 65536.f + 0.5f);
  a.drop_thresh = t > 65535u ? 65535u : t;
  a.drop_key = lowbias32_h(seed);
  a.drop_scale = 1.f / (1.f - drop_p);
  hipStream_t s = as_stream(stream);
// ... 44 lines not shown
```

### phantom_vlb_amd/csrc/ops.hip

```cpp
#include "common.hpp"

namespace {

constexpr int kMaxBlocks = 256 * 8;

__device__ __forceinline__ void load8(const bf16* p, float (&v)[8]) {
  const bf16x8 t = *reinterpret_cast<const bf16x8*>(p);
#pragma unroll
  for (int i = 0; i < 8; ++i) v[i] = (float)t[i];
}
__device__ __forceinline__ void store8(bf16* p, const float (&v)[8]) {
  bf16x8 t;
#pragma unroll
  for (int i = 0; i < 8; ++i) t[i] = (bf16)v[i];
  *reinterpret_cast<bf16x8*>(p) = t;
}

__global__ __launch_bounds__(256) void rmsnorm_fwd_kernel(const bf16* __restrict__ x, const bf16* __restrict__ w,
                                                          bf16* __restrict__ y, int rows, int dim, float eps) {
  const int row = blockIdx.x * 4 + (threadIdx.x >> 6), lane = threadIdx.x & 63;
  if (row >= rows) return;
  const bf16* xr = x + (int64_t)row * dim;
  float ss = 0.f;
  for (int c = lane * 8; c < dim; c += 512) {
// ... 175 lines not shown
  const float mean = wave_sum(s) / dim;
  float ss = 0.f;
#pragma unroll
  for (int k = 0; k < NI; ++k) {
    if (lane * 8 + k * 512 < dim) {
#pragma unroll
      for (int i = 0; i < 8; ++i) { const float d = (float)xb[k][i] - mean; ss += d * d; }
    }
  }
  const float rstd = rsqrtf(wave_sum(ss) / dim + eps);
  bf16* yr = y + (int64_t)row * dim;
#pragma unroll
  for (int k = 0; k < NI; ++k) {
    const int c = lane * 8 + k * 512;
    if (c < dim) {
      float v[8], g[8], bb[8]; load8(w + c, g); load8(b + c, bb);
#pragma unroll
      for (int i = 0; i < 8; ++i) v[i] = ((float)xb[k][i] - mean) * rstd * g[i] + bb[i];
      if (res) {
#pragma unroll
        for (int i = 0; i < 8; ++i) v[i] += (float)rb[k][i];
      }
      if (act != VLB_ACT_NONE) {
#pragma unroll
        for (int i = 0; i < 8; ++i) v[i] = act_f(v[i], act);
      }
      store8(yr + c, v);
    }
  }
}

__global__ __launch_bounds__(256) void layernorm_fwd_kernel(const bf16* __restrict__ x, const bf16* __restrict__ w,
                                                            const bf16* __restrict__ b, const bf16* __restrict__ res,
                                                            bf16* __restrict__ y, int rows, int dim, float eps, int act) {
  const int row = blockIdx.x * 4 + (threadIdx.x >> 6), lane = threadIdx.x & 63;
  if (row >= rows) return;
  const bf16* xr = x + (int64_t)row * dim;
  float s = 0.f;
  for (int c = lane * 8; c < dim; c += 512) {
    float v[8]; load8(xr + c, v);
#pragma unroll
    for (int i = 0; i < 8; ++i) s += v[i];
  }
  const float mean = wave_sum(s) / dim;
  float ss = 0.f;
  for (int c = lane * 8; c < dim; c += 512) {
    float v[8]; load8(xr + c, v);
#pragma unroll
    for (int i = 0; i < 8; ++i) { const float d = v[i] - mean; ss += d * d; }
  }
  const float rstd = rsqrtf(wave_sum(ss) / dim + eps);
  bf16* yr = y + (int64_t)row * dim;
  for (int c = lane * 8; c < dim; c += 512) {
    float v[8], g[8], bb[8]; load8(xr + c, v); load8(w + c, g); load8(b + c, bb);
#pragma unroll
    for (int i = 0; i < 8; ++i) v[i] = (v[i] - mean) * rstd * g[i] + bb[i];
    if (res) {
      float r[8]; load8(res + (int64_t)row * dim + c, r);
#pragma unroll
      for (int i = 0; i < 8; ++i) v[i] += r[i];
    }
    if (act != VLB_ACT_NONE) {
#pragma unroll
      for (int i = 0; i < 8; ++i) v[i] = act_f(v[i], act);
    }
    store8(yr + c, v);
  }
}

__global__ void rope_kernel(bf16* __restrict__ x, int ld, const float* __restrict__ cs, const float* __restrict__ sn,
                            int S, int heads, int D, float sign, const int* __restrict__ pos, int64_t total) {
  const int half = D >> 1, cpr = half >> 3;
  for (int64_t idx = blockIdx.x * (int64_t)blockDim.x + threadIdx.x; idx < total; idx += (int64_t)gridDim.x * blockDim.x) {
    const int ch = idx % cpr;
    const int h = (idx / cpr) % heads;
    const int64_t tok = idx / ((int64_t)cpr * heads);
    const int s = pos ? pos[tok] : (int)(tok % S);
    bf16* p = x + tok * ld + h * D + ch * 8;
    float a[8], b[8]; load8(p, a); load8(p + half, b);
    const float* c = cs + (int64_t)s * half + ch * 8;
    const float* n = sn + (int64_t)s * half + ch * 8;
    float oa[8], ob[8];
#pragma unroll
    for (int i = 0; i < 8; ++i) {
      const float co = c[i], si = sign * n[i];
      oa[i] = a[i] * co - b[i] * si;
      ob[i] = b[i] * co + a[i] * si;
    }
    store8(p, oa); store8(p + half, ob);
  }
}

__global__ void swiglu_fwd_kernel(const bf16* __restrict__ gu, bf16* __restrict__ out, int ff, int64_t total) {
  const int cpr = ff >> 3;
  for (int64_t idx = blockIdx.x * (int64_t)blockDim.x + threadIdx.x; idx < total; idx += (int64_t)gridDim.x * blockDim.x) {
    const int64_t r = idx / cpr; const int c = (idx % cpr) * 8;
    float g[8], u[8]; load8(gu + r * 2 * ff + c, g); load8(gu + r * 2 * ff + ff + c, u);
#pragma unroll
    for (int i = 0; i < 8; ++i) g[i] = silu_f(g[i]) * u[i];
    store8(out + r * ff + c, g);
  }
}
__global__ void swiglu_fwd_q8_kernel(const bf16* __restrict__ gu, bf16* __restrict__ out, uint8_t* __restrict__ q, int ldq,
                                     uint8_t* __restrict__ s, int lds_, int ff, int64_t total) {
  const int cpr = ff >> 3;
  for (int64_t idx = blockIdx.x * (int64_t)blockDim.x + threadIdx.x; idx < total; idx += (int64_t)gridDim.x * blockDim.x) {
    const int64_t r = idx / cpr; const int c = (idx % cpr) * 8;
    float g[8], u[8]; load8(gu + r * 2 * ff + c, g); load8(gu + r * 2 * ff + ff + c, u);
#pragma unroll
    for (int i = 0; i < 8; ++i) g[i] = (float)(bf16)(silu_f(g[i]) * u[i]);
    store8(out + r * ff + c, g);
    mx_quantize_lane8(g, q + r * ldq, s + r * lds_, c, threadIdx.x & 63);
  }
}
__global__ void swiglu_bwd_kernel(const bf16* __restrict__ gu, const bf16* __restrict__ dout, bf16* __restrict__ dgu,
                                  int ff, int64_t total) {
  const int cpr = ff >> 3;
  for (int64_t idx = blockIdx.x * (int64_t)blockDim.x + threadIdx.x; idx < total; idx += (int64_t)gridDim.x * blockDim.x) {
    const int64_t r = idx / cpr; const int c = (idx % cpr) * 8;
    float g[8], u[8], d[8], dg[8], du[8];
    load8(gu + r * 2 * ff + c, g); load8(gu + r * 2 * ff + ff + c, u); load8(dout + r * ff + c, d);
#pragma unroll
    for (int i = 0; i < 8; ++i) {
      const float sg = sigmoid_f(g[i]);
      const float si = g[i] * sg;
      du[i] = d[i] * si;
      dg[i] = d[i] * u[i] * (sg * (1.f + g[i] * (1.f - sg)));
    }
    store8(dgu + r * 2 * ff + c, dg); store8(dgu + r * 2 * ff + ff + c, du);
  }
}
__global__ void add_kernel(const bf16* __restrict__ a, const bf16* __restrict__ b, bf16* __restrict__ y, int64_t n8) {
  for (int64_t idx = blockIdx.x * (int64_t)blockDim.x + threadIdx.x; idx < n8; idx += (int64_t)gridDim.x * blockDim.x) {
    float x[8], z[8]; load8(a + idx * 8, x); load8(b + idx * 8, z);
#pragma unroll
    for (int i = 0; i < 8; ++i) x[i] += z[i];
    store8(y + idx * 8, x);
  }
}

__global__ void patchify_kernel(const float* __restrict__ vis, bf16* __restrict__ out, int H, int W, int P, int Kpad,
                                int64_t total) {
  const int G = W / P, GH = H / P, K = 3 * P * P, cpr = Kpad >> 3;
  for (int64_t idx = blockIdx.x * (int64_t)blockDim.x + threadIdx.x; idx < total; idx += (int64_t)gridDim.x * blockDim.x) {
    const int kc = (idx % cpr) * 8;
    const int64_t prow = idx / cpr;
    const int gx = prow % G, gy = (prow / G) % GH;
    const int64_t n = prow / ((int64_t)G * GH);
    float v[8];
#pragma unroll
    for (int i = 0; i < 8; ++i) {
      const int k = kc + i;
      if (k < K) {
        const int c = k / (P * P), py = (k / P) % P, px = k % P;
        v[i] = vis[((n * 3 + c) * H + gy * P + py) * (int64_t)W + gx * P + px];
      } else {
        v[i] = 0.f;
      }
    }
    store8(out + prow * Kpad + kc, v);
  }
}
__global__ void vit_assemble_kernel(const bf16* __restrict__ pe, const bf16* __restrict__ cls, const bf16* __restrict__ pos,
                                    bf16* __restrict__ tok, int G, int D, int64_t total) {
  const int cpr = D >> 3;
  for (int64_t idx = blockIdx.x * (int64_t)blockDim.x + threadIdx.x; idx < total; idx += (int64_t)gridDim.x * blockDim.x) {
    const int c = (idx % cpr) * 8;
    const int t = (idx / cpr) % (G + 1);
    const int64_t n = idx / ((int64_t)cpr * (G + 1));
    float a[8], p[8];
    if (t == 0) load8(cls + c, a); else load8(pe + (n * G + t - 1) * D + c, a);
// ... 533 lines not shown
```

### phantom_vlb_amd/fullft.py

```python
from __future__ import annotations

import os

import numpy as np
import torch

from . import ops
from ._lib import check, lib
from .flat import SEG_ALIGN
from .geometry import Geometry, VIDEO_TOKEN_ID

BF16 = torch.bfloat16
CONN_W = ("conv1", "dw", "se1", "se1b", "se2", "se2b", "conv3", "ds")
CONN_LN = ("bn1", "bn2", "bn3", "dsbn")


def _stream():
    return torch.cuda.current_stream().cuda_stream


FUSED_QUANT = os.environ.get("VLB_FP8_FUSED_QUANT", "1") == "1"


def _up(n, m):
    return (n + m - 1) // m * m


class FlatBackbone:

    grad_bf16 = True

    def __init__(self, g: Geometry, w):
        self.g = g
        slots = []

        def slot(name, holder, key, seg, idx=None):
            if idx is None:
                slots.append((name, holder[key], lambda t, h=holder, k=key: h.__setitem__(k, t), seg))
            else:
                def setter(t, h=holder, k=key, i=idx):
                    pair = list(h[k]); pair[i] = t; h[k] = tuple(pair)
                slots.append((name, holder[key][idx], setter, seg))
        for st, blocks in (("s1", w.s1), ("s2", w.s2)):
            for bi, blk in enumerate(blocks):
                for k in CONN_W:
                    if k in blk:
                        slot(f"mm_projector.{st}.b{bi + 1}.{k}", blk, k, -1)
                for k in CONN_LN:
                    if k in blk:
                        slot(f"mm_projector.{st}.b{bi + 1}.{k}.weight", blk, k, -1, 0)
                        slot(f"mm_projector.{st}.b{bi + 1}.{k}.bias", blk, k, -1, 1)
        wd = w.__dict__
        slot("mm_projector.sampler.weight", wd, "sampler_w", -1)
        slot("mm_projector.sampler.bias", wd, "sampler_b", -1)
        for k in ("ro0", "ro2"):
            slot(f"mm_projector.{k}.weight", wd, k, -1, 0)
            slot(f"mm_projector.{k}.bias", wd, k, -1, 1)
        slot("embed_tokens", wd, "embed", -1)
        slot("norm", wd, "final_norm", -1)
        for li, lw in enumerate(w.layers):
            for k in ("wqkv", "wo", "wgu", "wdown", "in_norm", "post_norm"):
                slot(f"layers.{li}.{k}", lw, k, li)
        offs, off, seg_start = {}, 0, 0
        self.layer_ranges = []
        for i, (name, t, _, seg) in enumerate(slots):
            offs[name] = (off, t.numel(), tuple(t.shape))
            off += _up(t.numel(), 8)
            if i + 1 == len(slots) or slots[i + 1][3] != seg:
                off = _up(off, SEG_ALIGN)
                if seg < 0:
                    self.head_range = (seg_start, off)
                else:
                    self.layer_ranges.append((seg_start, off))
                seg_start = off
        self.numel, self.offsets = off, offs
        dev = w.dev
        self.compute = torch.zeros(off, dtype=BF16, device=dev)
        self._setters = {}
        for name, t, setter, seg in slots:
            o, k, shp = offs[name]
            v = self.compute[o:o + k].view(shp)
            v.copy_(t)
            setter(v)
            self._setters[name] = (setter, seg)
        self.layers_released = False
        self.layer_grad_provider = None
        del slots
        torch.cuda.empty_cache()
        self.master = torch.empty(off, dtype=torch.float32, device=dev)
        step = 1 << 28
        for a in range(0, off, step):
            self.master[a:a + step].copy_(self.compute[a:a + step])
        self.grad = torch.zeros(off, dtype=BF16, device=dev)
        self.m = torch.zeros(off, dtype=torch.float32, device=dev)
        self.v = torch.zeros(off, dtype=torch.float32, device=dev)

    LAYER_KEYS = ("wqkv", "wo", "wgu", "wdown", "in_norm", "post_norm")

    def view(self, buf, name):
        o, k, shp = self.offsets[name]
        if o + k > buf.numel():
            raise RuntimeError(f"{name}: this store holds the tail segment only (FULL_SHARD) - layer tensors are reached through "
                               f"parallel.ShardedFlatState.layer_weights / layer_grads / gather_full")
        return buf[o:o + k].view(shp)
# ... 264 lines not shown
            self.wgrad(dysc, sv["x"], G(f"{pre}.ds"), xT=xT)
        if not need_dx:
            return None
        if dysc is not None:
            dx = ops.gemm(dy1, self.conn_t[f"{st}.{bi}.conv1"])
            return ops.gemm(dysc, self.conn_t[f"{st}.{bi}.ds"], residual=dx)
        return ops.gemm(dy1, self.conn_t[f"{st}.{bi}.conv1"], residual=dsc)

    def connector_backward(self, d_vid):
        g, w, sv, G = self.g, self.w, self.conn_saved, self.flat.g_
        B = sv["B"]
        self.wgrad(d_vid, sv["t1"], G("mm_projector.ro2.weight"))
        ops.colsum(d_vid, G("mm_projector.ro2.bias"))
        d_t1 = ops.gemm(d_vid, self.conn_t["ro2"])
        d_t0 = ops.act_bwd(sv["t0"], d_t1, ops.ACT_GELU)
        self.wgrad(d_t0, sv["ro_in"], G("mm_projector.ro0.weight"))
        ops.colsum(d_t0, G("mm_projector.ro0.bias"))
        dx = ops.gemm(d_t0, self.conn_t["ro0"])
        for bi in range(len(w.s2) - 1, -1, -1):
            dx = self._block_bwd(dx, w.s2[bi], "s2", bi, sv["s2"][bi], True)
        d_ypre = ops.act_bwd(sv["ypre"], dx, ops.ACT_SILU)
        self.wgrad(d_ypre, sv["cols"], G("mm_projector.sampler.weight"))
        ops.colsum(d_ypre, G("mm_projector.sampler.bias"))
        dcols = ops.gemm(d_ypre, self.conn_t["sampler"])
        dx = ops.col2im3d(dcols, B, g.num_frames, g.grid, g.grid, g.dim)
        for bi in range(len(w.s1) - 1, -1, -1):
            dx = self._block_bwd(dx, w.s1[bi], "s1", bi, sv["s1"][bi], bi > 0)
        self.conn_saved = None

    def forward(self, vision_f32, ids, layout=None, ids_host=None):
        g, bb, w = self.g, self.bb, self.w
        B = vision_f32.shape[0]
        vid = self.connector_forward(bb.video_tokens(vision_f32, tower_only=True), B)
        x, key_mask = bb.splice(ids, vid, layout)
        self._ids_host = ids_host if ids_host is not None else ids.cpu()
        S = g.max_len
        pos = None if layout is None else layout.pos
        qd, kd = g.heads * g.head_dim, g.kv_heads * g.head_dim
        self.saved = []
        for li in range(g.layers):
            lw = self._enter(li, backward=False)
            h1, h1q = self._norm(x, lw["in_norm"])
            qkv = self._lin(h1, li, "wqkv", xq=h1q)
            ops.rope_(qkv, w.rope_cos, w.rope_sin, B, S, g.heads + g.kv_heads, g.head_dim, pos=pos)
            a, lse = ops.attention_fwd(qkv[:, :qd], qkv[:, qd:qd + kd], qkv[:, qd + kd:], B, S, g.heads, g.kv_heads, g.head_dim,
                                       True, g.head_dim ** -0.5, key_mask=key_mask, need_lse=True, layout=layout)
            x2 = self._lin(a, li, "wo", residual=x)
            h2, h2q = self._norm(x2, lw["post_norm"])
            gu = self._lin(h2, li, "wgu", xq=h2q)
            if self.fp8 and FUSED_QUANT and gu.shape[1] % 64 == 0:
                hh, hq, hs = ops.swiglu_mxfp8(gu)
                x3 = self._lin(hh, li, "wdown", residual=x2, xq=(hq, hs))
            else:
                hh = ops.swiglu(gu)
                x3 = self._lin(hh, li, "wdown", residual=x2)
            self.saved.append(dict(x=x, h1=h1, qkv=qkv, a=a, lse=lse, x2=x2, h2=h2, gu=gu, hh=hh))
            x = x3
        self.x_last, self.key_mask, self.B, self.layout = x, key_mask, B, layout
        return ops.rmsnorm(x, w.final_norm, g.rms_eps), key_mask

    def backward(self, dhidden):
        g, w, G = self.g, self.w, self.flat.g_
        B, S = self.B, g.max_len
        qd, kd = g.heads * g.head_dim, g.kv_heads * g.head_dim
        layout = self.layout
        pos = None if layout is None else layout.pos
        dx = ops.rmsnorm_bwd_full(self.x_last, w.final_norm, dhidden, g.rms_eps, G("norm"))
        delta = torch.empty(B, g.heads, S, dtype=torch.float32, device=self.dev)
        for li in range(g.layers - 1, -1, -1):
            lw, sv = self._enter(li, backward=True), self.saved[li]
            pre = f"layers.{li}"
            dq_ = self._dual(dx) or (None, None)
            self.wgrad(dx, sv["hh"], G(f"{pre}.wdown"), fp8=self.fp8, dyTq=dq_[1])
            d_hh = self._lin(dx, li, "wdown_t", xq=dq_[0])
            d_gu = ops.swiglu_bwd(sv["gu"], d_hh)
            dq_ = self._dual(d_gu) or (None, None)
            self.wgrad(d_gu, sv["h2"], G(f"{pre}.wgu"), fp8=self.fp8, dyTq=dq_[1])
            d_h2 = self._lin(d_gu, li, "wgu_t", xq=dq_[0])
            dx2 = ops.rmsnorm_bwd_full(sv["x2"], lw["post_norm"], d_h2, g.rms_eps, G(f"{pre}.post_norm"), dx_in=dx)
            dq_ = self._dual(dx2) or (None, None)
            self.wgrad(dx2, sv["a"], G(f"{pre}.wo"), fp8=self.fp8, dyTq=dq_[1])
            d_a = self._lin(dx2, li, "wo_t", xq=dq_[0])
            dqkv = ops.attention_bwd(sv["qkv"], qd, kd, sv["a"], d_a, sv["lse"], self.key_mask, B, S, g.heads, g.kv_heads,
                                     g.head_dim, True, g.head_dim ** -0.5, layout=layout, delta=delta)
            ops.rope_(dqkv, w.rope_cos, w.rope_sin, B, S, g.heads + g.kv_heads, g.head_dim, sign=-1, pos=pos)
            dq_ = self._dual(dqkv) or (None, None)
            self.wgrad(dqkv, sv["h1"], G(f"{pre}.wqkv"), fp8=self.fp8, dyTq=dq_[1])
            d_h1 = self._lin(dqkv, li, "wqkv_t", xq=dq_[0])
            dx = ops.rmsnorm_bwd_full(sv["x"], lw["in_norm"], d_h1, g.rms_eps, G(f"{pre}.in_norm"), dx_in=dx2)
            self.saved[li] = None
            if self.grad_hook is not None:
                self.grad_hook(li)
        self._splice_backward(dx)
        self.saved = []

    def _splice_backward(self, d_embeds):
        g = self.g
        ids = self._ids_host.numpy() if torch.is_tensor(self._ids_host) else np.asarray(self._ids_host)
        B, L = ids.shape
        Nv, S = g.vis_tokens, g.max_len
        layout = self.layout
        lens = layout.lens if (layout is not None and layout.packed) else [S] * B
        cu = np.concatenate([[0], np.cumsum(lens)]) if (layout is not None and layout.packed) else np.arange(B + 1) * S
        tok_rows, tok_ids, vid_rows = [], [], []
        for b in range(B):
            vpos = int(np.nonzero(ids[b] == VIDEO_TOKEN_ID)[0][0])
            j = np.arange(L)
            p = np.where(j < vpos, j, j + Nv - 1)
            keep = (j != vpos) & (p < lens[b])
            tok_rows.append(cu[b] + p[keep])
            tok_ids.append(ids[b][keep])
            vid_rows.append(cu[b] + vpos + np.arange(Nv))
        tok_rows, tok_ids = np.concatenate(tok_rows), np.concatenate(tok_ids)
        order = np.lexsort((tok_rows, tok_ids))
        tok_rows, tok_ids = tok_rows[order], tok_ids[order]
        uniq, first = np.unique(tok_ids, return_index=True)
        beg = np.concatenate([first, [len(tok_ids)]])
        dev = self.dev
        i32 = lambda a: torch.from_numpy(np.ascontiguousarray(a, dtype=np.int32)).to(dev)
        dE = self.flat.g_("embed_tokens")
        dE.zero_()
        ops.embed_grad(d_embeds, i32(uniq), i32(beg), i32(tok_rows), dE, g.dim)
        vr = np.concatenate(vid_rows)
        d_vid = torch.empty(B * Nv, g.dim, dtype=BF16, device=dev)
        n = B * Nv
        ops.embed_grad(d_embeds, i32(np.arange(n)), i32(np.arange(n + 1)), i32(vr), d_vid, g.dim)
        self.connector_backward(d_vid)

    def state_dict(self, which: str = "master") -> dict:
        g, f = self.g, self.flat
        buf = getattr(f, which)
        if self.shards is not None and (buf is None or buf.numel() < f.numel):
            buf = self.shards.gather_full(which)
        M = lambda n: f.view(buf, n).detach().float().cpu()
        qd, kd = g.heads * g.head_dim, g.kv_heads * g.head_dim
        sd = {"model.embed_tokens.weight": M("embed_tokens"), "model.norm.weight": M("norm")}
        for li in range(g.layers):
            p, q = f"model.layers.{li}", f"layers.{li}"
            wqkv, wgu = M(f"{q}.wqkv"), M(f"{q}.wgu")
            sd[f"{p}.self_attn.q_proj.weight"] = wqkv[:qd].clone()
            sd[f"{p}.self_attn.k_proj.weight"] = wqkv[qd:qd + kd].clone()
            sd[f"{p}.self_attn.v_proj.weight"] = wqkv[qd + kd:].clone()
            sd[f"{p}.self_attn.o_proj.weight"] = M(f"{q}.wo")
            sd[f"{p}.mlp.gate_proj.weight"] = wgu[:g.ff].clone()
            sd[f"{p}.mlp.up_proj.weight"] = wgu[g.ff:].clone()
            sd[f"{p}.mlp.down_proj.weight"] = M(f"{q}.wdown")
            sd[f"{p}.input_layernorm.weight"] = M(f"{q}.in_norm")
            sd[f"{p}.post_attention_layernorm.weight"] = M(f"{q}.post_norm")
        P = "model.mm_projector"
        for st, blocks in (("s1", self.w.s1), ("s2", self.w.s2)):
            for bi, blk in enumerate(blocks):
                q, n = f"{P}.{st}.b{bi + 1}", f"mm_projector.{st}.b{bi + 1}"
                C = blk["conv1"].shape[0]
                sd[f"{q}.conv1.conv.weight"] = M(f"{n}.conv1")[:, :, None, None].clone()
                sd[f"{q}.conv2.conv.weight"] = M(f"{n}.dw").t().reshape(C, 1, 3, 3).clone()
                sd[f"{q}.conv3.conv.weight"] = M(f"{n}.conv3")[:, :, None, None].clone()
                for k, u in (("se1", "se.fc1"), ("se2", "se.fc2")):
                    sd[f"{q}.{u}.weight"] = M(f"{n}.{k}")[:, :, None, None].clone()
                    sd[f"{q}.{u}.bias"] = M(f"{n}.{k}b")
                for k, u in (("bn1", "conv1.bn"), ("bn2", "conv2.bn"), ("bn3", "conv3.bn")):
                    sd[f"{q}.{u}.weight"], sd[f"{q}.{u}.bias"] = M(f"{n}.{k}.weight"), M(f"{n}.{k}.bias")
                if "ds" in blk:
                    sd[f"{q}.downsample.conv.weight"] = M(f"{n}.ds")[:, :, None, None].clone()
                    sd[f"{q}.downsample.bn.weight"], sd[f"{q}.downsample.bn.bias"] = M(f"{n}.dsbn.weight"), M(f"{n}.dsbn.bias")
        sw = M("mm_projector.sampler.weight")
        C = sw.shape[0]
        sd[f"{P}.sampler.0.weight"] = sw.view(C, 2, 2, 2, C).permute(0, 4, 1, 2, 3).contiguous()
        sd[f"{P}.sampler.0.bias"] = M("mm_projector.sampler.bias")
# ... 4 lines not shown
```

### phantom_vlb_amd/lora.py

```python
from __future__ import annotations

import ctypes
import math

import torch

from . import ops
from ._lib import check, lib
from .geometry import Geometry

BF16 = torch.bfloat16
PAD = 64
FUSE_SWIGLU_BWD = True
MERGE_DB_U = True


def _stream():
    return torch.cuda.current_stream().cuda_stream


def _seeds(vals):
    return (ctypes.c_uint32 * len(vals))(*[v & 0xFFFFFFFF for v in vals])


def lora_down(x, A, R, scale, p, seeds, out):
    M, K = x.shape
    check(lib.vlb_lora_down(x.data_ptr(), x.stride(0), A.data_ptr(), out.data_ptr(), out.stride(0), M, K, R, scale, p,
                            _seeds(seeds) if p > 0 else None, _stream()), "vlb_lora_down")
    return out


def lora_dx_masked(u, At, dx, R, p, seeds):
    M, K = dx.shape
    check(lib.vlb_lora_dx_masked(u.data_ptr(), u.stride(0), At.data_ptr(), At.stride(0), dx.data_ptr(), dx.stride(0), M, K, R, p,
                                 _seeds(seeds), _stream()), "vlb_lora_dx_masked")


def wgrad_skinny_u(G, X, dW, ws, Bt, u_scale, u_out, u_ws, alpha=1.0, beta=0.0):
    M, K = X.shape
    check(lib.vlb_wgrad_skinny_u(G.data_ptr(), G.stride(0), X.data_ptr(), X.stride(0), dW.data_ptr(), ws.data_ptr(), M, K,
                                 alpha, beta, Bt.data_ptr(), u_scale, u_out.data_ptr(), u_out.stride(0), u_ws.data_ptr(),
                                 _stream()), "vlb_wgrad_skinny_u")


def wgrad_skinny_u_multi(G, X, cols, dWs, Bts, ws, u_scale, u_out, u_ws, alpha=1.0, beta=0.0):
    M = X.shape[0]
    n = len(cols)
    check(lib.vlb_wgrad_skinny_u_multi(G.data_ptr(), G.stride(0), X.data_ptr(), X.stride(0), M, n, (ctypes.c_int * n)(*cols),
                                       (ctypes.c_void_p * n)(*[t.data_ptr() for t in dWs]), (ctypes.c_void_p * n)(*[t.data_ptr() for t in Bts]),
                                       ws.data_ptr(), alpha, beta, u_scale, u_out.data_ptr(), u_out.stride(0), u_ws.data_ptr(), _stream()),
          "vlb_wgrad_skinny_u_multi")


def wgrad_skinny(G, X, dW, ws, N, alpha=1.0, beta=0.0, p=0.0, seeds=None):
    M, K = X.shape
    check(lib.vlb_wgrad_skinny(G.data_ptr(), G.stride(0), X.data_ptr(), X.stride(0), dW.data_ptr(), ws.data_ptr(), M, N, K,
                               alpha, beta, p, _seeds(seeds) if p > 0 else None, _stream()), "vlb_wgrad_skinny")


GROUPS = (
    ("qkv", ("self_attn.q_proj", "self_attn.k_proj", "self_attn.v_proj")),
    ("o", ("self_attn.o_proj",)),
    ("gu", ("mlp.gate_proj", "mlp.up_proj")),
    ("down", ("mlp.down_proj",)),
)


class LoraState:
    def __init__(self, g: Geometry, weights, r: int, alpha: int, dropout: float, device, seed: int = 1234,
                 sd: dict | None = None, target_modules=None):
        if not isinstance(r, int) or not 1 <= r <= 64:
            raise NotImplementedError(f"lora_r={r}: ranks 1..64 are built (up to four 16-wide MFMA tiles per adapted projection); "
                                      "the reference's setting is 16 (config/experiment/VLB_vllama2_friends_lora.yaml:27)")
        want = sorted(t.split(".")[-1] for _, ts in GROUPS for t in ts)
        if target_modules is not None and sorted(target_modules) != want:
            raise NotImplementedError(f"LoRA target_modules {sorted(target_modules)}: the adapted decoder is built for "
                                      f"exactly {want}")
        self.g, self.w, self.r, self.dev = g, weights, r, device
        self.gu_il = "wgu_il" in weights.layers[0]
        self.c = c = (r + 15) // 16
        self.rp = rp = 16 * c
        self.scale = alpha / r
        self.p = float(dropout)
        self.step = 0
        self.rank = 0
        self.grad_hook = None
        self.base_seed = seed
        qd, kd = g.heads * g.head_dim, g.kv_heads * g.head_dim
        self.out_dims = {"self_attn.q_proj": qd, "self_attn.k_proj": kd, "self_attn.v_proj": kd, "self_attn.o_proj": g.dim,
                         "mlp.gate_proj": g.ff, "mlp.up_proj": g.ff, "mlp.down_proj": g.dim}
        self.in_dims = {"self_attn.q_proj": g.dim, "self_attn.k_proj": g.dim, "self_attn.v_proj": g.dim,
                        "self_attn.o_proj": qd, "mlp.gate_proj": g.dim, "mlp.up_proj": g.dim, "mlp.down_proj": g.ff}
        gen = torch.Generator(device="cpu").manual_seed(seed + 17)
        self.master: dict[str, torch.Tensor] = {}
        self.grads: dict[str, torch.Tensor] = {}
        self.layers = []
# ... 58 lines not shown
            return self._jobs
        rec = []
        for i, lay in enumerate(self.layers):
            for gname, targets in GROUPS:
                blk = lay[gname]
                row = 0
                for j, t in enumerate(targets):
                    pre = f"model.layers.{i}.{t}"
                    a, bt = cc[f"{pre}.lora_A.weight"], cc[f"{pre}.lora_B.weight"]
                    for b in range(self.c):
                        col = self.rp * j + 16 * b
                        il = int(self.gu_il and gname == "gu")
                        brow = 16 * j if il else row
                        for src, dst, n, mode in ((a[16 * b:16 * b + 16], blk["At"][:, col:], a.shape[1], 0),
                                                  (bt[16 * b:16 * b + 16], blk["Bpad"][brow:, col:], bt.shape[1], il)):
                            assert src.is_contiguous() and src.shape[0] == 16 and dst.stride(0) == blk["Rpad"]
                            for n0 in range(0, n, 256):
                                rec.append(struct.pack("<QQiiii", src.data_ptr(), dst.data_ptr(), n, n0, blk["Rpad"], mode))
                    row += self.out_dims[t]
        buf = torch.frombuffer(bytearray(b"".join(rec)), dtype=torch.uint8).to(self.dev)
        self._jobs, self._jobs_key, self._n_jobs = buf, key, len(rec)
        return buf

    def refresh(self, from_master=False):
        if from_master:
            cc = self.compute_copies()
            for n, t in cc.items():
                t.copy_(self.master[n])
        jobs = self._scatter_jobs()
        check(lib.vlb_transpose16_scatter(jobs.data_ptr(), self._n_jobs, _stream()), "vlb_transpose16_scatter")

    def state_dict(self):
        r = self.r
        return {n: (t[:r].t().contiguous() if "lora_B" in n else t[:r].clone()) for n, t in self.master.items()}

    def load_state_dict(self, sd: dict):
        r = self.r
        for n, t in self.master.items():
            src = sd[n].to(self.dev, torch.float32)
            t[:r].copy_(src.t() if "lora_B" in n else src)
        self.refresh(from_master=True)

    def _seed(self, layer, target_idx):
        x = (self.base_seed * 0x9E3779B1 + self.step * 0x85EBCA6B + layer * 0xC2B2AE35 + target_idx * 0x27D4EB2F
             + self.rank * 0x7F4A7C15) & 0xFFFFFFFF
        return x or 1

    def _workspace(self, M):
        if self._ws is None or self._ws["cap"] < M:
            g, d = self.g, self.dev
            kmax = max(g.ff, g.dim, g.heads * g.head_dim)
            kgrp = max(2 * g.ff, (g.heads + 2 * g.kv_heads) * g.head_dim)
            self._ws = dict(cap=M, wg=torch.empty(lib.vlb_wgrad_splits(M) * 48 * kmax, dtype=torch.float32, device=d),
                            uws=torch.empty(lib.vlb_wgrad_u_ws_floats(M, kgrp), dtype=torch.float32, device=d),
                            u_full=torch.zeros(M, self._rpad_max(), dtype=BF16, device=d))
        self._ws["u"] = self._ws["u_full"][:M]
        return self._ws

    def _rpad_max(self):
        return max(blk["Rpad"] for blk in self.layers[0].values())

    def _group_seeds(self, seeds, n_targets):
        return None if seeds is None else [seeds[j] for j in range(n_targets) for _ in range(self.c)]

    def _t_buffer(self, li, gi, M):
        if getattr(self, "_t_cap", 0) < M:
            self._t_cap = M
            self._t_bufs = torch.zeros(len(self.layers), len(GROUPS), M, self._rpad_max(), dtype=BF16, device=self.dev)
        return self._t_bufs[li, gi, :M, :self.layers[li][GROUPS[gi][0]]["Rpad"]]

    def _lora_t(self, x, blk, seeds, slot=None, p=None):
        t = self._t_buffer(*slot, x.shape[0]) if slot is not None else torch.zeros(x.shape[0], blk["Rpad"], dtype=BF16, device=self.dev)
        p = self.p if p is None else p
        gs = self._group_seeds(seeds, len(blk["targets"])) if p > 0 else None
        for r0 in range(0, blk["R"], 48):
            n = min(48, blk["R"] - r0)
            lora_down(x, blk["A"][r0:r0 + n], n, self.scale, p, None if gs is None else gs[r0 // 16:(r0 + n) // 16], t[:, r0:])
        return t

    def _adapted(self, x, W, blk, seeds, residual=None, slot=None, p=None):
        t = self._lora_t(x, blk, seeds, slot, p)
        return ops.gemm(x, W, residual=residual, a2=t, w2=blk["Bpad"]), t

    def _adapted_mlp_in(self, x, lw, blk, seeds, slot, p=None, save=True):
        if self.gu_il:
            t = self._lora_t(x, blk, seeds, slot, p)
            if save:
                hh, gu = ops.gemm_swiglu_save(x, lw["wgu_il"], a2=t, w2_il=blk["Bpad"])
                return hh, gu, t
            return ops.gemm(x, lw["wgu_il"], act=ops.ACT_SWIGLU_PAIR, a2=t, w2=blk["Bpad"]), None, t
        gu, t = self._adapted(x, lw["wgu"], blk, seeds, slot=slot, p=p)
        return ops.swiglu(gu), gu, t

    def forward(self, backbone, vision_f32, ids, layout=None, train=True):
        g = self.g
        B = vision_f32.shape[0]
        vid = backbone.video_tokens(vision_f32)
        x, key_mask = backbone.splice(ids, vid, layout)
        return self.decoder_forward(backbone, x, key_mask, B, layout, train=train)

    def decoder_forward(self, backbone, x, key_mask, B, layout=None, train=True):
        g, w = self.g, self.w
        S = g.max_len
        pos = None if layout is None else layout.pos
        qd, kd = g.heads * g.head_dim, g.kv_heads * g.head_dim
        if not train:
            return self._decoder_eval(backbone, x, key_mask, B, layout)
        self.saved = []
        self.step += 1
        for li, lay in enumerate(self.layers):
            lw = backbone.layer_weights(li)
            sd = [self._seed(li, k) for k in range(7)]
            h1 = ops.rmsnorm(x, lw["in_norm"], g.rms_eps)
            qkv, t_qkv = self._adapted(h1, lw["wqkv"], lay["qkv"], sd[0:3], slot=(li, 0))
            ops.rope_(qkv, w.rope_cos, w.rope_sin, B, S, g.heads + g.kv_heads, g.head_dim, pos=pos)
            a, lse = ops.attention_fwd(qkv[:, :qd], qkv[:, qd:qd + kd], qkv[:, qd + kd:], B, S, g.heads, g.kv_heads,
                                       g.head_dim, True, g.head_dim ** -0.5, key_mask=key_mask, need_lse=True,
                                       layout=layout)
            x2, t_o = self._adapted(a, lw["wo"], lay["o"], sd[3:4], residual=x, slot=(li, 1))
            h2 = ops.rmsnorm(x2, lw["post_norm"], g.rms_eps)
            hh, gu, t_gu = self._adapted_mlp_in(h2, lw, lay["gu"], sd[4:6], (li, 2))
            x3, t_d = self._adapted(hh, lw["wdown"], lay["down"], sd[6:7], residual=x2, slot=(li, 3))
            self.saved.append(dict(x=x, h1=h1, qkv=qkv, a=a, lse=lse, x2=x2, h2=h2, gu=gu, hh=hh, t_qkv=t_qkv, t_o=t_o,
                                   t_gu=t_gu, t_d=t_d, seeds=sd))
            x = x3
        self.x_last, self.key_mask, self.B, self.layout = x, key_mask, B, layout
        return ops.rmsnorm(x, w.final_norm, g.rms_eps), key_mask

    def _decoder_eval(self, backbone, x, key_mask, B, layout):
        g, w = self.g, self.w
        S = g.max_len
        pos = None if layout is None else layout.pos
        qd, kd = g.heads * g.head_dim, g.kv_heads * g.head_dim
        for li, lay in enumerate(self.layers):
            lw = backbone.layer_weights(li)
            h = ops.rmsnorm(x, lw["in_norm"], g.rms_eps)
            qkv, _ = self._adapted(h, lw["wqkv"], lay["qkv"], None, slot=(li, 0), p=0.0)
            ops.rope_(qkv, w.rope_cos, w.rope_sin, B, S, g.heads + g.kv_heads, g.head_dim, pos=pos)
            a = ops.attention_fwd(qkv[:, :qd], qkv[:, qd:qd + kd], qkv[:, qd + kd:], B, S, g.heads, g.kv_heads, g.head_dim,
                                  True, g.head_dim ** -0.5, key_mask=key_mask, layout=layout)
            x, _ = self._adapted(a, lw["wo"], lay["o"], None, residual=x, slot=(li, 1), p=0.0)
            h = ops.rmsnorm(x, lw["post_norm"], g.rms_eps)
            hh, _, _ = self._adapted_mlp_in(h, lw, lay["gu"], None, (li, 2), p=0.0, save=False)
            x, _ = self._adapted(hh, lw["wdown"], lay["down"], None, residual=x, slot=(li, 3), p=0.0)
        return ops.rmsnorm(x, w.final_norm, g.rms_eps), key_mask

    def _group_backward(self, li, gname, dy, x_in, t, seeds, W_t, need_dx, swiglu_gu=None):
        lay = self.layers[li][gname]
        ws = self._workspace(dy.shape[0])
        u = ws["u"]
        col = 0
        u = u[:, :lay["Rpad"]]
        rp = self.rp
        names = [f"model.layers.{li}.{tname}" for tname in lay["targets"]]
        cols = [self.out_dims[tname] for tname in lay["targets"]]
        multi = MERGE_DB_U and self.c == 1 and len(cols) > 1 and all(n % 256 == 0 for n in cols) and dy.shape[1] == sum(cols)
        if multi:
            wgrad_skinny_u_multi(t, dy, cols, [self.grads[f"{pre}.lora_B.weight"] for pre in names],
                                 [self.bt[f"{pre}.lora_B.weight"] for pre in names], ws["wg"], self.scale, u, ws["uws"])
        for j, tname in enumerate(() if multi else lay["targets"]):
            n = self.out_dims[tname]
            pre = f"model.layers.{li}.{tname}"
            dyj = dy[:, col:col + n]
            for b in range(self.c):
                k = rp * j + 16 * b
                wgrad_skinny_u(t[:, k:k + 16], dyj, self.grads[f"{pre}.lora_B.weight"][16 * b:16 * b + 16], ws["wg"],
                               self.bt[f"{pre}.lora_B.weight"][16 * b:16 * b + 16], self.scale, u[:, k:k + 16], ws["uws"])
            col += n
        gs = self._group_seeds(seeds, len(lay["targets"])) if self.p > 0 else None
        for r0 in range(0, lay["R"], 48):
            n = min(48, lay["R"] - r0)
            wgrad_skinny(u[:, r0:], x_in, self.grad_A[li][gname][r0:r0 + n], ws["wg"], n, p=self.p,
                         seeds=None if gs is None else gs[r0 // 16:(r0 + n) // 16])
        if not need_dx:
            return None
        if self.p == 0.0:
            dx = ops.gemm(dy, W_t, a2=u, w2=lay["At"])
        elif lay["R"] == 16 and ops.gemm_masked_pair_ok(dy.shape[0], W_t.shape[0], dy.shape[1]):
            if swiglu_gu is not None and FUSE_SWIGLU_BWD:
                return ops.gemm_masked_pair_swiglu_bwd(dy, W_t, swiglu_gu, u, lay["At"], self.p, seeds[0])
            dx = ops.gemm_masked_pair(dy, W_t, u, lay["At"], self.p, seeds[0])
        else:
            dx = ops.gemm(dy, W_t)
            for r0 in range(0, lay["R"], 48):
                n = min(48, lay["R"] - r0)
                lora_dx_masked(u[:, r0:], lay["At"][:, r0:], dx, n, self.p, gs[r0 // 16:(r0 + n) // 16])
        return dx if swiglu_gu is None else ops.swiglu_bwd(swiglu_gu, dx)

    def backward(self, backbone, dhidden):
        g, w = self.g, self.w
        B, S = self.B, g.max_len
        qd, kd = g.heads * g.head_dim, g.kv_heads * g.head_dim
        layout = self.layout
        pos = None if layout is None else layout.pos
        M = self.x_last.shape[0]
        dx = ops.rmsnorm_bwd(self.x_last, w.final_norm, dhidden, g.rms_eps)
        delta = torch.empty(B, g.heads, S, dtype=torch.float32, device=self.dev)
        for li in range(g.layers - 1, -1, -1):
            lw, sv = backbone.layer_weights(li, transposed=True, direction=-1), self.saved[li]
            sd = sv["seeds"]
            d_gu = self._group_backward(li, "down", dx, sv["hh"], sv["t_d"], sd[6:7], lw["wdown_t"], True, swiglu_gu=sv["gu"])
            d_h2 = self._group_backward(li, "gu", d_gu, sv["h2"], sv["t_gu"], sd[4:6], lw["wgu_t"], True)
            dx2 = ops.rmsnorm_bwd(sv["x2"], lw["post_norm"], d_h2, g.rms_eps, dx_in=dx)
            d_a = self._group_backward(li, "o", dx2, sv["a"], sv["t_o"], sd[3:4], lw["wo_t"], True)
            qkv = sv["qkv"]
            dqkv = ops.attention_bwd(qkv, qd, kd, sv["a"], d_a, sv["lse"], self.key_mask, B, S, g.heads, g.kv_heads,
                                     g.head_dim, True, g.head_dim ** -0.5, layout=layout, delta=delta)
            ops.rope_(dqkv, w.rope_cos, w.rope_sin, B, S, g.heads + g.kv_heads, g.head_dim, sign=-1, pos=pos)
            need_dx = li > 0
            d_h1 = self._group_backward(li, "qkv", dqkv, sv["h1"], sv["t_qkv"], sd[0:3], lw["wqkv_t"], need_dx)
            if need_dx:
                dx = ops.rmsnorm_bwd(sv["x"], lw["in_norm"], d_h1, g.rms_eps, dx_in=dx2)
            if self.grad_hook is not None:
                self.grad_hook(li)
        self.saved = []
```

### phantom_vlb_amd/ops.py

```python
from __future__ import annotations

import torch

from ._lib import check, lib

ACT_NONE, ACT_QUICK_GELU, ACT_GELU, ACT_SILU, ACT_SWIGLU_PAIR = 0, 1, 2, 3, 4
BF16 = torch.bfloat16


def _stream():
    return torch.cuda.current_stream().cuda_stream


def _p(t):
    return None if t is None else t.data_ptr()


def _dev(t):
    if not t.is_cuda:
        raise RuntimeError("phantom_vlb_amd ops need GPU tensors (no CPU fallback)")
    return t


class _GemmProbe:
# ... 15 lines not shown
        torch.cuda.synchronize()
        out = {}
        for kind, flops, e0, e1 in self.calls:
            c = out.setdefault(kind, [0, 0.0, 0.0])
            c[0] += 1
            c[1] += e0.elapsed_time(e1)
            c[2] += flops / 1e12
        return out


_probe = None


def enable_gemm_probe(N, K, family=False):
    global _probe
    _probe = _GemmProbe(N, K, family)
    return _probe


def disable_gemm_probe():
    global _probe
    _probe = None


class _Timed:

    def __init__(self, kind, M, N, K, K2=0):
        pr = _probe
        self.e = None
        if pr is None:
            return
        shape = N == pr.N and K == pr.K and kind != "masked"
        fam = pr.family and K + K2 >= 4096
        if not (shape or fam):
            return
        self.e = (torch.cuda.Event(enable_timing=True), torch.cuda.Event(enable_timing=True))
        if shape and not pr.family:
            pr.M = M
            pr.pairs.append(self.e)
        if fam:
            pr.calls.append((kind, 2.0 * M * N * (K + K2)) + self.e)

    def __enter__(self):
        if self.e:
            self.e[0].record()

    def __exit__(self, *a):
        if self.e:
            self.e[1].record()


_gemm_ws = {}
split_k_tails = True


def _gemm_workspace(device):
    if not split_k_tails:
        return None
    key = (device.index, torch.cuda.current_stream(device).cuda_stream)
    ws = _gemm_ws.get(key)
    if ws is None:
        ws = _gemm_ws[key] = torch.empty(lib.vlb_gemm_workspace_bytes(), dtype=torch.uint8, device=device)
    return ws


def gemm(a, w, bias=None, residual=None, act=ACT_NONE, a2=None, w2=None, out=None):
    _dev(a)
    M, K = a.shape
    N = w.shape[0]
    assert w.shape[1] == K and a.stride(1) == 1 and w.stride(1) == 1
    if out is None:
        out = torch.empty(M, N // 2 if act == ACT_SWIGLU_PAIR else N, dtype=BF16, device=a.device)
    K2 = 0
    if a2 is not None:
        K2 = a2.shape[1]
        assert w2.shape == (N, K2) and a2.shape[0] == M
    ws = _gemm_workspace(a.device) if K + K2 >= 4096 and M * N > 256 * 192 * 256 else None
    with _Timed("plain", M, N, K, K2):
        check(lib.vlb_gemm_bf16_ws(a.data_ptr(), a.stride(0), w.data_ptr(), w.stride(0), out.data_ptr(), out.stride(0),
                                   M, N, K, _p(bias), _p(residual), residual.stride(0) if residual is not None else 0, act,
                                   _p(a2), a2.stride(0) if a2 is not None else 0, _p(w2),
                                   w2.stride(0) if w2 is not None else 0, K2, _p(ws), ws.numel() if ws is not None else 0,
                                   _stream()), "vlb_gemm_bf16")
    return out


def gemm_swiglu_save(a, w_il, a2=None, w2_il=None):
    _dev(a)
    M, K = a.shape
    N = w_il.shape[0]
    assert w_il.shape[1] == K and a.stride(1) == 1 and w_il.stride(1) == 1 and N % 32 == 0
    h = torch.empty(M, N // 2, dtype=BF16, device=a.device)
    gu = torch.empty(M, N, dtype=BF16, device=a.device)
    K2 = 0
    if a2 is not None:
        K2 = a2.shape[1]
        assert w2_il.shape == (N, K2) and a2.shape[0] == M
    ws = _gemm_workspace(a.device) if K + K2 >= 4096 and M * N > 256 * 192 * 256 else None
    with _Timed("gate_up+swiglu", M, N, K, K2):
        check(lib.vlb_gemm_swiglu_save(a.data_ptr(), a.stride(0), w_il.data_ptr(), w_il.stride(0), h.data_ptr(), h.stride(0),
                                       gu.data_ptr(), gu.stride(0), M, N, K, _p(a2), a2.stride(0) if a2 is not None else 0, _p(w2_il),
                                       w2_il.stride(0) if w2_il is not None else 0, K2, _p(ws), ws.numel() if ws is not None else 0,
                                       _stream()), "vlb_gemm_swiglu_save")
    return h, gu


def gemm_masked_pair_ok(M, N, K):
    return N % 256 == 0 and K % 64 == 0 and K >= 128 and M * (N // 2) < 2 ** 32


def gemm_masked_pair(a, w, a2, w2, p, seed, out=None):
    _dev(a)
    M, K = a.shape
    N = w.shape[0]
    assert w.shape[1] == K and a2.shape[0] == M and w2.shape[0] == N and a2.shape[1] >= 64 and w2.shape[1] >= 64
    if out is None:
        out = torch.empty(M, N, dtype=BF16, device=a.device)
    ws = _gemm_workspace(a.device) if K + 64 >= 4096 and M * N > 256 * 192 * 256 else None
    with _Timed("masked", M, N, K, 64):
        check(lib.vlb_gemm_bf16_masked_pair_ws(a.data_ptr(), a.stride(0), w.data_ptr(), w.stride(0), out.data_ptr(), out.stride(0),
                                               M, N, K, a2.data_ptr(), a2.stride(0), w2.data_ptr(), w2.stride(0), float(p),
                                               int(seed) & 0xFFFFFFFF, _p(ws), ws.numel() if ws is not None else 0, _stream()),
              "vlb_gemm_bf16_masked_pair")
    return out


def gemm_masked_pair_swiglu_bwd(dy, w_t, gu, a2, w2, p, seed, out=None):
    _dev(dy)
    M, K = dy.shape
    ff = w_t.shape[0]
    assert w_t.shape[1] == K and gu.shape == (M, 2 * ff) and a2.shape[0] == M and w2.shape[0] == ff
    if out is None:
        out = torch.empty(M, 2 * ff, dtype=BF16, device=dy.device)
    ws = _gemm_workspace(dy.device) if K + 64 >= 4096 and M * ff > 256 * 192 * 256 else None
    with _Timed("masked", M, ff, K, 64):
        check(lib.vlb_gemm_masked_pair_swiglu_bwd(dy.data_ptr(), dy.stride(0), w_t.data_ptr(), w_t.stride(0), gu.data_ptr(), gu.stride(0),
                                                  out.data_ptr(), out.stride(0), M, ff, K, a2.data_ptr(), a2.stride(0), w2.data_ptr(),
                                                  w2.stride(0), float(p), int(seed) & 0xFFFFFFFF, _p(ws),
                                                  ws.numel() if ws is not None else 0, _stream()), "vlb_gemm_masked_pair_swiglu_bwd")
    return out


def interleave_gate_up(w_gate, w_up):
    ff, k = w_gate.shape
    assert ff % 16 == 0
    return torch.stack([w_gate.view(ff // 16, 16, k), w_up.view(ff // 16, 16, k)], 1).reshape(2 * ff, k).contiguous()


def transpose(x):
    R, C = x.shape
    out = torch.empty(C, R, dtype=BF16, device=x.device)
    check(lib.vlb_transpose_bf16(_dev(x).data_ptr(), out.data_ptr(), R, C, _stream()), "vlb_transpose_bf16")
    return out


class RowLayout:

    def __init__(self, B, S, lens=None, device=None):
        self.B, self.S = int(B), int(S)
        if lens is None:
            self.cu = self.pos = self.lens = None
            self.rows, self.smax = self.B * self.S, self.S
            return
        lens = [int(x) for x in lens]
        if len(lens) != self.B or min(lens) < 1 or max(lens) > self.S:
            raise ValueError(f"RowLayout: lens {lens} do not fit B={B}, S={S}")
        cu = [0]
        for n in lens:
            cu.append(cu[-1] + n)
        self.lens, self.rows, self.smax = lens, cu[-1], max(lens)
        self.cu = torch.tensor(cu, dtype=torch.int32).to(device, non_blocking=True)
        self.pos = torch.empty(self.rows, dtype=torch.int32, device=device)

    @property
    def packed(self):
        return self.cu is not None

    def unpack(self, x, fill=0.0):
        if not self.packed:
            return x.view(self.B, self.S, -1)
        out = torch.full((self.B, self.S, x.shape[1]), fill, dtype=x.dtype, device=x.device)
        o = 0
        for b, n in enumerate(self.lens):
            out[b, :n] = x[o:o + n]
            o += n
        return out


def attention_fwd(q, k, v, B, S, Hq, Hkv, D, causal, scale, key_mask=None, need_lse=False, out=None, layout=None):
    _dev(q)
    cu, rows = None, B * S
    if layout is not None and layout.packed:
        B, S, cu, rows = layout.B, layout.smax, layout.cu, layout.rows
    assert q.shape[0] == rows, f"attention_fwd: {q.shape[0]} rows, layout has {rows}"
    if out is None:
        out = torch.empty(rows, Hq * D, dtype=BF16, device=q.device)
    lse = torch.empty(B, Hq, S, dtype=torch.float32, device=q.device) if need_lse else None
    check(lib.vlb_attention_fwd(q.data_ptr(), q.stride(0), k.data_ptr(), k.stride(0), v.data_ptr(), v.stride(0),
                                out.data_ptr(), out.stride(0), _p(lse), _p(key_mask), B, S, Hq, Hkv, D,
                                1 if causal else 0, float(scale), _p(cu), _stream()), "vlb_attention_fwd")
    return (out, lse) if need_lse else out


_ATTN_WS = [None]


def _attn_workspace(n_floats, device):
    ws = _ATTN_WS[0]
    if ws is None or ws.numel() < n_floats or ws.device != device:
        ws = _ATTN_WS[0] = torch.empty(n_floats, dtype=torch.float32, device=device)
    return ws


def attention_bwd(qkv, qd, kd, out, dout, lse, key_mask, B, S, Hq, Hkv, D, causal, scale, layout=None, delta=None,
                  dq_acc=None):
    cu, rows = None, B * S
    if layout is not None and layout.packed:
        B, S, cu, rows = layout.B, layout.smax, layout.cu, layout.rows
    assert qkv.shape[0] == rows and dout.shape[0] == rows
    if delta is None:
        delta = torch.empty(B, Hq, S, dtype=torch.float32, device=qkv.device)
    if dq_acc is None and Hq != Hkv:
        dq_acc = _attn_workspace(rows * qd, qkv.device)
    assert delta.numel() >= B * Hq * S and (dq_acc is None or dq_acc.numel() >= rows * qd)
    dqkv = torch.empty_like(qkv)
    check(lib.vlb_attention_bwd(qkv.data_ptr(), qkv.stride(0), qkv[:, qd:].data_ptr(), qkv.stride(0),
                                qkv[:, qd + kd:].data_ptr(), qkv.stride(0), out.data_ptr(), out.stride(0),
                                dout.data_ptr(), dout.stride(0), lse.data_ptr(), _p(key_mask),
                                dqkv.data_ptr(), dqkv.stride(0), dqkv[:, qd:].data_ptr(), dqkv.stride(0),
                                dqkv[:, qd + kd:].data_ptr(), dqkv.stride(0), delta.data_ptr(), _p(dq_acc),
                                B, S, Hq, Hkv, D, 1 if causal else 0, float(scale), _p(cu), rows, _stream()),
          "vlb_attention_bwd")
    return dqkv


def rmsnorm(x, w, eps, out=None):
    rows, dim = x.shape
    if out is None:
        out = torch.empty_like(x)
    check(lib.vlb_rmsnorm_fwd(_dev(x).data_ptr(), w.data_ptr(), out.data_ptr(), rows, dim, eps, _stream()), "vlb_rmsnorm_fwd")
    return out


def rmsnorm_bwd(x, w, dy, eps, dx_in=None, out=None):
    rows, dim = x.shape
    if out is None:
        out = torch.empty_like(x)
    check(lib.vlb_rmsnorm_bwd(_dev(x).data_ptr(), w.data_ptr(), dy.data_ptr(), _p(dx_in), out.data_ptr(), rows, dim, eps,
                              _stream()), "vlb_rmsnorm_bwd")
    return out


def layernorm(x, w, b, eps, residual=None, act=ACT_NONE, out=None):
    rows, dim = x.shape
    if out is None:
        out = torch.empty_like(x)
    check(lib.vlb_layernorm_fwd(_dev(x).data_ptr(), w.data_ptr(), b.data_ptr(), _p(residual), out.data_ptr(), rows, dim,
                                eps, act, _stream()), "vlb_layernorm_fwd")
    return out


def rope_(x, cos, sin, B, S, heads, D, sign=1, pos=None):
    rows = B * S if pos is None else pos.shape[0]
    assert x.shape[0] == rows and cos.shape[0] >= S
    check(lib.vlb_rope_inplace(_dev(x).data_ptr(), x.stride(0), cos.data_ptr(), sin.data_ptr(), rows, S, heads, D, sign,
                               _p(pos), _stream()), "vlb_rope_inplace")
    return x


def swiglu(gu, out=None):
    rows, ff2 = gu.shape
    if out is None:
        out = torch.empty(rows, ff2 // 2, dtype=BF16, device=gu.device)
    check(lib.vlb_swiglu_fwd(_dev(gu).data_ptr(), out.data_ptr(), rows, ff2 // 2, _stream()), "vlb_swiglu_fwd")
    return out


def swiglu_bwd(gu, dout, out=None):
    rows, ff2 = gu.shape
    if out is None:
        out = torch.empty_like(gu)
    check(lib.vlb_swiglu_bwd(_dev(gu).data_ptr(), dout.data_ptr(), out.data_ptr(), rows, ff2 // 2, _stream()), "vlb_swiglu_bwd")
    return out


def add(a, b, out=None):
    if out is None:
        out = torch.empty_like(a)
    check(lib.vlb_add_bf16(_dev(a).data_ptr(), b.data_ptr(), out.data_ptr(), a.numel(), _stream()), "vlb_add_bf16")
    return out


def patchify(vision_f32, P, Kpad):
    N, C, H, W = vision_f32.shape
    assert C == 3 and vision_f32.dtype == torch.float32 and vision_f32.is_contiguous()
    out = torch.empty(N * (H // P) * (W // P), Kpad, dtype=BF16, device=vision_f32.device)
    check(lib.vlb_patchify(_dev(vision_f32).data_ptr(), out.data_ptr(), N, H, W, P, Kpad, _stream()), "vlb_patchify")
    return out


def vit_assemble(patch_emb, cls, pos, N, G, D):
    out = torch.empty(N * (G + 1), D, dtype=BF16, device=patch_emb.device)
    check(lib.vlb_vit_assemble(_dev(patch_emb).data_ptr(), cls.data_ptr(), pos.data_ptr(), out.data_ptr(), N, G, D,
                               _stream()), "vlb_vit_assemble")
    return out


def drop_cls(tokens, N, G, D):
    out = torch.empty(N * G, D, dtype=BF16, device=tokens.device)
    check(lib.vlb_drop_cls(_dev(tokens).data_ptr(), out.data_ptr(), N, G, D, _stream()), "vlb_drop_cls")
    return out


def dwconv3x3(x, w9, N, H, W, C):
    out = torch.empty_like(x)
# ... 231 lines not shown
```

Measured before the change: 15.01 clips/s.

## Fuse RoPE into QKV GEMM epilogue and attention backward, fold delta into dQ

Applies rotary embedding in the QKV projection GEMM epilogue instead of a separate in-place pass. In the attention backward, the inverse RoPE is applied inside the dQ kernel's store and inside the grouped dK/dV reduction. The delta (rowsum of O·dO) is computed inside the dQ kernel, which now runs before dK/dV, so the standalone delta kernel and its extra read of O and dO go away. The aim is to remove several full read/write passes over qkv/dqkv per layer. In exchange the code gains more template variants, a changed kernel order, and slightly different rounding in the dQ RoPE path.

```diff
diff --git a/include/vlb.h b/include/vlb.h
--- a/include/vlb.h
+++ b/include/vlb.h
@@ -21,6 +21,7 @@
 #define VLB_ACT_GELU 2
 #define VLB_ACT_SILU 3
 #define VLB_ACT_SWIGLU_PAIR 4
+#define VLB_ACT_ROPE_QK 6
 #define VLB_ACT_SWIGLU_BWD 5
 
 int vlb_abi_version(void);
@@ -36,6 +37,9 @@
 int vlb_gemm_swiglu_save(const void* A, int lda, const void* W_il, int ldw, void* H, int ldh, void* GU, int ldgu, int M, int N,
                          int K, const void* A2, int lda2, const void* W2_il, int ldw2, int K2, void* ws, int64_t ws_bytes,
                          void* stream);
+int vlb_gemm_rope_qk(const void* A, int lda, const void* W, int ldw, void* C, int ldc, int M, int N, int K, const void* A2,
+                     int lda2, const void* W2, int ldw2, int K2, const float* cos_t, const float* sin_t, const int* pos,
+                     int rope_S, int rope_cols, void* ws, int64_t ws_bytes, void* stream);
 int64_t vlb_gemm_workspace_bytes(void);
 int vlb_gemm_plan(int M, int N, int K, int K2, int with_workspace);
 
@@ -64,6 +68,12 @@
                       int lddq, void* dk, int lddk, void* dv, int lddv, float* delta, float* dq_acc, int B, int S,
                       int Hq, int Hkv, int D, int causal, float scale, const int* cu_rows, int total_rows,
                       void* stream);
+int vlb_attention_bwd_fused(const void* q, int ldq, const void* k, int ldk, const void* v, int ldv, const void* out,
+                            int ldo, const void* dout, int lddo, const float* lse, const uint8_t* key_mask, void* dq,
+                            int lddq, void* dk, int lddk, void* dv, int lddv, float* delta, float* dq_acc, int B, int S,
+                            int Hq, int Hkv, int D, int causal, float scale, const int* cu_rows, int total_rows,
+                            int fuse_delta, const float* cos_t, const float* sin_t, const int* pos, int rope_S,
+                            void* stream);
 
 int vlb_rmsnorm_fwd(const void* x, const void* w, void* y, int rows, int dim, float eps, void* stream);
 int vlb_rmsnorm_bwd(const void* x, const void* w, const void* dy, const void* dx_in, void* dx, int rows, int dim,
diff --git a/phantom_vlb_amd/_lib.py b/phantom_vlb_amd/_lib.py
--- a/phantom_vlb_amd/_lib.py
+++ b/phantom_vlb_amd/_lib.py
@@ -18,12 +18,14 @@
     "vlb_gemm_bf16": [P, I, P, I, P, I, I, I, I, P, P, I, I, P, I, P, I, I, P],
     "vlb_gemm_bf16_ws": [P, I, P, I, P, I, I, I, I, P, P, I, I, P, I, P, I, I, P, L, P],
     "vlb_gemm_swiglu_save": [P, I, P, I, P, I, P, I, I, I, I, P, I, P, I, I, P, L, P],
+    "vlb_gemm_rope_qk": [P, I, P, I, P, I, I, I, I, P, I, P, I, I, P, P, P, I, I, P, L, P],
     "vlb_gemm_workspace_bytes": [],
     "vlb_gemm_plan": [I, I, I, I, I],
     "vlb_gemm_kernel_choice": [I, I, I, I],
     "vlb_transpose_bf16": [P, P, I, I, P],
     "vlb_attention_fwd": [P, I, P, I, P, I, P, I, P, P, I, I, I, I, I, I, F, P, P],
     "vlb_attention_bwd": [P, I, P, I, P, I, P, I, P, I, P, P, P, I, P, I, P, I, P, P, I, I, I, I, I, I, F, P, I, P],
+    "vlb_attention_bwd_fused": [P, I, P, I, P, I, P, I, P, I, P, P, P, I, P, I, P, I, P, P, I, I, I, I, I, I, F, P, I, I, P, P, P, I, P],
     "vlb_rmsnorm_fwd": [P, P, P, I, I, F, P],
     "vlb_rmsnorm_bwd": [P, P, P, P, P, I, I, F, P],
     "vlb_layernorm_fwd": [P, P, P, P, P, I, I, F, I, P],
diff --git a/phantom_vlb_amd/csrc/attention.hip b/phantom_vlb_amd/csrc/attention.hip
--- a/phantom_vlb_amd/csrc/attention.hip
+++ b/phantom_vlb_amd/csrc/attention.hip
@@ -288,6 +288,13 @@
 
 __device__ __forceinline__ int sw2(int r) { return ((r & 3) << 2) | ((r >> 2) & 3); }
 
+__device__ __forceinline__ float delta_chunk(const bf16x8 a, const bf16x8 b) {
+  float s = 0.f;
+#pragma unroll
+  for (int i = 0; i < 8; ++i) s = __fadd_rn(s, __fmul_rn((float)a[i], (float)b[i]));
+  return s;
+}
+
 __global__ __launch_bounds__(256) void attn_delta_kernel(const bf16* __restrict__ o, int ldo, const bf16* __restrict__ d_o,
                                                          int lddo, float* __restrict__ delta, int S, int Hq, int B,
                                                          const int* __restrict__ cu, int64_t total) {
@@ -298,8 +305,7 @@
     const int h = gid % Hq; const int64_t tok = gid / Hq;
     const bf16x8 a = *reinterpret_cast<const bf16x8*>(o + tok * ldo + h * 128 + c * 8);
     const bf16x8 b = *reinterpret_cast<const bf16x8*>(d_o + tok * lddo + h * 128 + c * 8);
-#pragma unroll
-    for (int i = 0; i < 8; ++i) s += (float)a[i] * (float)b[i];
+    s = delta_chunk(a, b);
   }
 #pragma unroll
   for (int off = 8; off > 0; off >>= 1) s += __shfl_xor(s, off, 64);
@@ -504,6 +510,44 @@
   *reinterpret_cast<bf16x8*>(dst + hkv * 128 + c * 8) = o;
 }
 
+__global__ __launch_bounds__(256) void attn_dkdv_reduce_rope_kernel(const bf16* __restrict__ part, bf16* __restrict__ dk, int lddk,
+                                                                    bf16* __restrict__ dv, int lddv, int Hq, int Hkv,
+                                                                    const float* __restrict__ cs, const float* __restrict__ sn,
+                                                                    const int* __restrict__ pos, int rope_S, int64_t total) {
+  const int64_t i = blockIdx.x * (int64_t)blockDim.x + threadIdx.x;
+  if (i >= total) return;
+  const int c = i & 7, which = (i >> 3) & 1;
+  const int hkv = (int)((i >> 4) % Hkv);
+  const int64_t row = (i >> 4) / Hkv;
+  const int gsz = Hq / Hkv;
+  float lo[8] = {0.f, 0.f, 0.f, 0.f, 0.f, 0.f, 0.f, 0.f}, hi[8] = {0.f, 0.f, 0.f, 0.f, 0.f, 0.f, 0.f, 0.f};
+  const bf16* src = part + (row * Hq + (int64_t)hkv * gsz) * 256 + which * 128 + c * 8;
+  for (int j = 0; j < gsz; ++j) {
+    const bf16x8 v = *reinterpret_cast<const bf16x8*>(src + (int64_t)j * 256);
+    const bf16x8 w = *reinterpret_cast<const bf16x8*>(src + (int64_t)j * 256 + 64);
+#pragma unroll
+    for (int e = 0; e < 8; ++e) { lo[e] += (float)v[e]; hi[e] += (float)w[e]; }
+  }
+  bf16x8 o, q;
+#pragma unroll
+  for (int e = 0; e < 8; ++e) { o[e] = (bf16)lo[e]; q[e] = (bf16)hi[e]; }
+  if (which == 0) {
+    const int s = pos ? pos[row] : (int)(row % rope_S);
+    const f32x4* cp = reinterpret_cast<const f32x4*>(cs + (int64_t)s * 64 + c * 8);
+    const f32x4* sp = reinterpret_cast<const f32x4*>(sn + (int64_t)s * 64 + c * 8);
+    const f32x4 c0 = cp[0], c1 = cp[1], s0 = sp[0], s1 = sp[1];
+#pragma unroll
+    for (int e = 0; e < 8; ++e) {
+      float ra, rb;
+      rope_pair((float)o[e], (float)q[e], e < 4 ? c0[e & 3] : c1[e & 3], e < 4 ? s0[e & 3] : s1[e & 3], -1.f, ra, rb);
+      o[e] = (bf16)ra; q[e] = (bf16)rb;
+    }
+  }
+  bf16* dst = (which ? dv + row * lddv : dk + row * lddk) + hkv * 128 + c * 8;
+  *reinterpret_cast<bf16x8*>(dst) = o;
+  *reinterpret_cast<bf16x8*>(dst + 64) = q;
+}
+
 struct AttnDqArgs {
   const bf16* q; const bf16* k; const bf16* v; const bf16* dout;
   const float* lse; const float* delta; const uint8_t* mask; const int* cu;
@@ -511,9 +555,11 @@
   int ldq, ldk, ldv, lddo, lddq;
   int B, S, Hq, Hkv;
   float scale;
+  const bf16* out; int ldo; float* delta_w;
+  const float* cs; const float* sn; const int* pos; int rope_S;
 };
 
-template <bool CAUSAL>
+template <bool CAUSAL, bool DELTA, bool ROPE>
 __global__ __launch_bounds__(256, 2) void attn_bwd_dq_kernel(AttnDqArgs p) {
   constexpr int D = 128, ROWB = 256, TILE = KV * ROWB, KS = 8, DT = 4;
   extern __shared__ __attribute__((aligned(16))) char smem[];
@@ -544,7 +590,19 @@
     }
   }
   const float lse_q = p.lse[((int64_t)b * p.Hq + hq) * p.S + qr];
-  const float delta_q = p.delta[((int64_t)b * p.Hq + hq) * p.S + qr];
+  float delta_q;
+  if constexpr (DELTA) {
+    const bf16* op = p.out + (row0 + qr) * p.ldo + hq * D + 8 * h;
+    float sc[KS];
+#pragma unroll
+    for (int ks = 0; ks < KS; ++ks) sc[ks] = delta_chunk(*reinterpret_cast<const bf16x8*>(op + 16 * ks), dof[ks]);
+    const float t = __fadd_rn(__fadd_rn(__fadd_rn(sc[0], sc[4]), __fadd_rn(sc[2], sc[6])),
+                              __fadd_rn(__fadd_rn(sc[1], sc[5]), __fadd_rn(sc[3], sc[7])));
+    delta_q = __fadd_rn(t, __shfl_xor(t, 32, 64));
+    if (h == 0 && qrow < Sb) p.delta_w[((int64_t)b * p.Hq + hq) * p.S + qrow] = delta_q;
+  } else {
+    delta_q = p.delta[((int64_t)b * p.Hq + hq) * p.S + qr];
+  }
   const float c2 = p.scale * 1.44269504088896341f;
   const float lse2 = (lse_q > -1e37f) ? lse_q * 1.44269504088896341f : 1e37f;
 
@@ -664,25 +722,62 @@
 
   if (qrow < Sb) {
     bf16* op = p.dq + (row0 + qrow) * p.lddq + hq * D;
-#pragma unroll
-    for (int dt = 0; dt < DT; ++dt)
-#pragma unroll
-      for (int g = 0; g < 4; ++g) {
-        bf16x4 o;
-#pragma unroll
-        for (int e = 0; e < 4; ++e) o[e] = (bf16)dqt[dt][4 * g + e];
-        *reinterpret_cast<bf16x4*>(op + 32 * dt + 8 * g + 4 * h) = o;
-      }
-  }
-}
-
-}
-
-extern "C" int vlb_attention_bwd(const void* q, int ldq, const void* k, int ldk, const void* v, int ldv, const void* out,
-                                 int ldo, const void* dout, int lddo, const float* lse, const uint8_t* key_mask, void* dq,
-                                 int lddq, void* dk, int lddk, void* dv, int lddv, float* delta, float* dq_acc, int B,
-                                 int S, int Hq, int Hkv, int D, int causal, float scale, const int* cu_rows, int total_rows,
-                                 void* stream) {
+    if constexpr (ROPE) {
+      const int64_t tok = row0 + qrow;
+      const int s = p.pos ? p.pos[tok] : (int)(tok % p.rope_S);
+      const float* cp = p.cs + (int64_t)s * (D / 2) + 4 * h;
+      const float* sp = p.sn + (int64_t)s * (D / 2) + 4 * h;
+#pragma unroll
+      for (int dt = 0; dt < DT / 2; ++dt)
+#pragma unroll
+        for (int g = 0; g < 4; ++g) {
+          const f32x4 co = *reinterpret_cast<const f32x4*>(cp + 32 * dt + 8 * g);
+          const f32x4 si = *reinterpret_cast<const f32x4*>(sp + 32 * dt + 8 * g);
+          bf16x4 oa, ob;
+#pragma unroll
+          for (int e = 0; e < 4; ++e) {
+            float ra, rb;
+            rope_pair((float)(bf16)dqt[dt][4 * g + e], (float)(bf16)dqt[dt + 2][4 * g + e], co[e], si[e], -1.f, ra, rb);
+            oa[e] = (bf16)ra; ob[e] = (bf16)rb;
+          }
+          *reinterpret_cast<bf16x4*>(op + 32 * dt + 8 * g + 4 * h) = oa;
+          *reinterpret_cast<bf16x4*>(op + 64 + 32 * dt + 8 * g + 4 * h) = ob;
+        }
+    } else {
+#pragma unroll
+      for (int dt = 0; dt < DT; ++dt)
+#pragma unroll
+        for (int g = 0; g < 4; ++g) {
+          bf16x4 o;
+#pragma unroll
+          for (int e = 0; e < 4; ++e) o[e] = (bf16)dqt[dt][4 * g + e];
+          *reinterpret_cast<bf16x4*>(op + 32 * dt + 8 * g + 4 * h) = o;
+        }
+    }
+  }
+}
+
+}
+
+namespace {
+
+template <bool DELTA, bool ROPE>
+int launch_dq(const AttnDqArgs& d, dim3 grid, bool causal, hipStream_t st) {
+  constexpr int LDS_DQ = 2 * 2 * KV * 256;
+  static const hipError_t q1 = hipFuncSetAttribute(reinterpret_cast<const void*>(&attn_bwd_dq_kernel<true, DELTA, ROPE>), hipFuncAttributeMaxDynamicSharedMemorySize, LDS_DQ);
+  static const hipError_t q2 = hipFuncSetAttribute(reinterpret_cast<const void*>(&attn_bwd_dq_kernel<false, DELTA, ROPE>), hipFuncAttributeMaxDynamicSharedMemorySize, LDS_DQ);
+  if (q1 != hipSuccess || q2 != hipSuccess) { vlb_set_error("attention_bwd: LDS reservation failed (dq)"); return VLB_ERR_LAUNCH; }
+  if (causal) hipLaunchKernelGGL((attn_bwd_dq_kernel<true, DELTA, ROPE>), grid, dim3(256), LDS_DQ, st, d);
+  else hipLaunchKernelGGL((attn_bwd_dq_kernel<false, DELTA, ROPE>), grid, dim3(256), LDS_DQ, st, d);
+  VLB_LAUNCH_CHECK();
+  return VLB_OK;
+}
+
+int attention_bwd_impl(const void* q, int ldq, const void* k, int ldk, const void* v, int ldv, const void* out, int ldo,
+                       const void* dout, int lddo, const float* lse, const uint8_t* key_mask, void* dq, int lddq, void* dk,
+                       int lddk, void* dv, int lddv, float* delta, float* dq_acc, int B, int S, int Hq, int Hkv, int D,
+                       int causal, float scale, const int* cu_rows, int total_rows, bool fuse_delta, const float* cos_t,
+                       const float* sin_t, const int* pos, int rope_S, void* stream) {
   VLB_REQUIRE(q && k && v && out && dout && lse && dq && dk && dv && delta, "attention_bwd: null operand");
   VLB_REQUIRE(dq_acc || Hq == Hkv, "attention_bwd: the [rows, Hq, D] fp32-sized workspace is required");
   VLB_REQUIRE(D == 128, "attention_bwd: head dim %d unsupported (only 128: the decoder)", D);
@@ -691,20 +786,36 @@
                   lddk % 4 == 0 && lddv % 4 == 0, "attention_bwd: strides must keep vector alignment");
   VLB_REQUIRE(((((uintptr_t)q | (uintptr_t)k | (uintptr_t)v | (uintptr_t)out | (uintptr_t)dout) % 16) == 0) &&
                   ((uintptr_t)dq % 8 == 0), "attention_bwd: misaligned pointer");
+  const bool rope = cos_t != nullptr;
+  VLB_REQUIRE(!rope || (sin_t && rope_S > 0 && (((uintptr_t)cos_t | (uintptr_t)sin_t) % 16) == 0),
+              "attention_bwd: rope tables must be 16-byte aligned fp32 [S, 64] with S > 0");
   hipStream_t st = as_stream(stream);
   const int64_t rows = cu_rows ? (int64_t)total_rows : (int64_t)B * S;
   VLB_REQUIRE(rows > 0 && rows <= (int64_t)B * S, "attention_bwd: total_rows=%d out of range", total_rows);
-  const int64_t th = rows * Hq;
-  hipLaunchKernelGGL(attn_delta_kernel, dim3((unsigned)((th + 15) / 16)), dim3(256), 0, st, (const bf16*)out, ldo,
-                     (const bf16*)dout, lddo, delta, S, Hq, B, cu_rows, th);
-  VLB_LAUNCH_CHECK();
+  const int gsz = Hq / Hkv;
+  VLB_REQUIRE(gsz == 1 || dq_acc, "attention_bwd: the workspace (fp32 [rows, Hq, D]) is required for grouped-query heads");
+  VLB_REQUIRE(lddk % 8 == 0 && lddv % 8 == 0 && (((uintptr_t)dk | (uintptr_t)dv) % 16) == 0, "attention_bwd: dk/dv rows must be 16-byte aligned");
+
+  AttnDqArgs d{(const bf16*)q, (const bf16*)k, (const bf16*)v, (const bf16*)dout, lse, delta, key_mask, cu_rows,
+               (bf16*)dq, ldq, ldk, ldv, lddo, lddq, B, S, Hq, Hkv, scale, (const bf16*)out, ldo, delta, cos_t, sin_t, pos, rope_S};
+  const dim3 gq(((S + QB - 1) / QB) * Hq * B);
+  auto run_dq = [&]() {
+    if (fuse_delta) return rope ? launch_dq<true, true>(d, gq, causal, st) : launch_dq<true, false>(d, gq, causal, st);
+    return rope ? launch_dq<false, true>(d, gq, causal, st) : launch_dq<false, false>(d, gq, causal, st);
+  };
+  if (fuse_delta) {
+    const int rc = run_dq();
+    if (rc != VLB_OK) return rc;
+  } else {
+    const int64_t th = rows * Hq;
+    hipLaunchKernelGGL(attn_delta_kernel, dim3((unsigned)((th + 15) / 16)), dim3(256), 0, st, (const bf16*)out, ldo,
+                       (const bf16*)dout, lddo, delta, S, Hq, B, cu_rows, th);
+    VLB_LAUNCH_CHECK();
+  }
   AttnBwdArgs a{(const bf16*)q, (const bf16*)k, (const bf16*)v, (const bf16*)dout, lse, delta, key_mask, cu_rows,
                 (bf16*)dk, (bf16*)dv, dq_acc, ldq, ldk, ldv, lddo, lddk, lddv, B, S, Hq, Hkv, scale, g_attn_ablate};
   dim3 grid((S + BK_KEYS - 1) / BK_KEYS, Hkv, B);
   {
-    const int gsz = Hq / Hkv;
-    VLB_REQUIRE(gsz == 1 || dq_acc, "attention_bwd: the workspace (fp32 [rows, Hq, D]) is required for grouped-query heads");
-    VLB_REQUIRE(lddk % 8 == 0 && lddv % 8 == 0 && (((uintptr_t)dk | (uintptr_t)dv) % 16) == 0, "attention_bwd: dk/dv rows must be 16-byte aligned");
     constexpr int LDS_KV = BK_KEYS * 256 + 4 * BQ * 256 + 512;
     static const hipError_t k1 = hipFuncSetAttribute(reinterpret_cast<const void*>(&attn_bwd_dkdv_kernel<true>), hipFuncAttributeMaxDynamicSharedMemorySize, LDS_KV);
     static const hipError_t k2 = hipFuncSetAttribute(reinterpret_cast<const void*>(&attn_bwd_dkdv_kernel<false>), hipFuncAttributeMaxDynamicSharedMemorySize, LDS_KV);
@@ -714,24 +825,45 @@
     if (causal) hipLaunchKernelGGL(attn_bwd_dkdv_kernel<true>, gridh, dim3(256), LDS_KV, st, a, part);
     else hipLaunchKernelGGL(attn_bwd_dkdv_kernel<false>, gridh, dim3(256), LDS_KV, st, a, part);
     VLB_LAUNCH_CHECK();
-    if (gsz > 1) {
+    if (gsz > 1 && rope) {
+      const int64_t tot = rows * Hkv * 16;
+      hipLaunchKernelGGL(attn_dkdv_reduce_rope_kernel, dim3((unsigned)((tot + 255) / 256)), dim3(256), 0, st, part, (bf16*)dk,
+                         lddk, (bf16*)dv, lddv, Hq, Hkv, cos_t, sin_t, pos, rope_S, tot);
+      VLB_LAUNCH_CHECK();
+    } else if (gsz > 1) {
       const int64_t tot = rows * Hkv * 32;
       hipLaunchKernelGGL(attn_dkdv_reduce_kernel, dim3((unsigned)((tot + 255) / 256)), dim3(256), 0, st, part, (bf16*)dk, lddk,
                          (bf16*)dv, lddv, Hq, Hkv, tot);
       VLB_LAUNCH_CHECK();
-    }
-  }
-  AttnDqArgs d{(const bf16*)q, (const bf16*)k, (const bf16*)v, (const bf16*)dout, lse, delta, key_mask, cu_rows,
-               (bf16*)dq, ldq, ldk, ldv, lddo, lddq, B, S, Hq, Hkv, scale};
-  constexpr int LDS_DQ = 2 * 2 * KV * 256;
-  static const hipError_t q1 = hipFuncSetAttribute(reinterpret_cast<const void*>(&attn_bwd_dq_kernel<true>), hipFuncAttributeMaxDynamicSharedMemorySize, LDS_DQ);
-  static const hipError_t q2 = hipFuncSetAttribute(reinterpret_cast<const void*>(&attn_bwd_dq_kernel<false>), hipFuncAttributeMaxDynamicSharedMemorySize, LDS_DQ);
-  if (q1 != hipSuccess || q2 != hipSuccess) { vlb_set_error("attention_bwd: LDS reservation failed (dq)"); return VLB_ERR_LAUNCH; }
-  dim3 gq(((S + QB - 1) / QB) * Hq * B);
-  if (causal) hipLaunchKernelGGL(attn_bwd_dq_kernel<true>, gq, dim3(256), LDS_DQ, st, d);
-  else hipLaunchKernelGGL(attn_bwd_dq_kernel<false>, gq, dim3(256), LDS_DQ, st, d);
-  VLB_LAUNCH_CHECK();
-  return VLB_OK;
+    } else if (rope) {
+      const int rc = vlb_rope_inplace(dk, lddk, cos_t, sin_t, (int)rows, rope_S, Hkv, D, -1, pos, stream);
+      if (rc != VLB_OK) return rc;
+    }
+  }
+  return fuse_delta ? VLB_OK : run_dq();
+}
+
+}
+
+extern "C" int vlb_attention_bwd(const void* q, int ldq, const void* k, int ldk, const void* v, int ldv, const void* out,
+                                 int ldo, const void* dout, int lddo, const float* lse, const uint8_t* key_mask, void* dq,
+                                 int lddq, void* dk, int lddk, void* dv, int lddv, float* delta, float* dq_acc, int B,
+                                 int S, int Hq, int Hkv, int D, int causal, float scale, const int* cu_rows, int total_rows,
+                                 void* stream) {
+  return attention_bwd_impl(q, ldq, k, ldk, v, ldv, out, ldo, dout, lddo, lse, key_mask, dq, lddq, dk, lddk, dv, lddv, delta,
+                            dq_acc, B, S, Hq, Hkv, D, causal, scale, cu_rows, total_rows, false, nullptr, nullptr, nullptr, 0,
+                            stream);
+}
+
+extern "C" int vlb_attention_bwd_fused(const void* q, int ldq, const void* k, int ldk, const void* v, int ldv, const void* out,
+                                       int ldo, const void* dout, int lddo, const float* lse, const uint8_t* key_mask,
+                                       void* dq, int lddq, void* dk, int lddk, void* dv, int lddv, float* delta, float* dq_acc,
+                                       int B, int S, int Hq, int Hkv, int D, int causal, float scale, const int* cu_rows,
+                                       int total_rows, int fuse_delta, const float* cos_t, const float* sin_t, const int* pos,
+                                       int rope_S, void* stream) {
+  return attention_bwd_impl(q, ldq, k, ldk, v, ldv, out, ldo, dout, lddo, lse, key_mask, dq, lddq, dk, lddk, dv, lddv, delta,
+                            dq_acc, B, S, Hq, Hkv, D, causal, scale, cu_rows, total_rows, fuse_delta != 0, cos_t, sin_t, pos,
+                            rope_S, stream);
 }
 
 #ifdef VLB_TOOLS
diff --git a/phantom_vlb_amd/csrc/common.hpp b/phantom_vlb_amd/csrc/common.hpp
--- a/phantom_vlb_amd/csrc/common.hpp
+++ b/phantom_vlb_amd/csrc/common.hpp
@@ -73,6 +73,12 @@
 __device__ __forceinline__ float quick_gelu_f(float x) { return x * sigmoid_f(1.702f * x); }
 __device__ __forceinline__ float gelu_erf_f(float x) { return 0.5f * x * (1.f + erff(x * 0.70710678118654752f)); }
 
+__device__ __forceinline__ void rope_pair(float a, float b, float co, float sn, float sign, float& oa, float& ob) {
+  const float si = __fmul_rn(sign, sn);
+  oa = __fmaf_rn(a, co, -__fmul_rn(b, si));
+  ob = __fmaf_rn(b, co, __fmul_rn(a, si));
+}
+
 __device__ __forceinline__ int mx_shared_exp(float amax) {
   int E = -127;
   if (amax > 0.f) {
diff --git a/phantom_vlb_amd/csrc/gemm.hip b/phantom_vlb_amd/csrc/gemm.hip
--- a/phantom_vlb_amd/csrc/gemm.hip
+++ b/phantom_vlb_amd/csrc/gemm.hip
@@ -24,6 +24,7 @@
   bf16* aux; int ldaux;
   int reserved;
   int wide;
+  const float* rope_cos; const float* rope_sin; const int* rope_pos; int rope_S, rope_cols;
 };
 
 __device__ __forceinline__ void tile_coords(const GemmArgs& p, int pid, int sub, int BM, int BN, int& m0, int& n0) {
@@ -682,6 +683,49 @@
     }
     return;
   }
+  if constexpr (NT == 8 && !MASKED) {
+    if (p.act == VLB_ACT_ROPE_QK) {
+      const int nb = n0 + wn * TN;
+      if (nb < p.rope_cols) {
+#pragma unroll
+        for (int i = 0; i < MT; ++i) {
+          const int m = m0 + wm * TM + i * 16 + fr;
+          if (m >= p.M) continue;
+          const int s = p.rope_pos ? p.rope_pos[m] : m % p.rope_S;
+          const float* cp = p.rope_cos + (int64_t)s * 64 + fq * 4;
+          const float* sp = p.rope_sin + (int64_t)s * 64 + fq * 4;
+          bf16* crow = p.C + (int64_t)m * p.ldc;
+#pragma unroll
+          for (int j = 0; j < 4; j += 2) {
+            bf16x4 lo[2], hi[2];
+#pragma unroll
+            for (int t = 0; t < 2; ++t) {
+              const f32x4 co = *reinterpret_cast<const f32x4*>(cp + (j + t) * 16);
+              const f32x4 si = *reinterpret_cast<const f32x4*>(sp + (j + t) * 16);
+#pragma unroll
+              for (int e = 0; e < 4; ++e) {
+                float ra, rb;
+                rope_pair((float)(bf16)acc[i][j + t][e], (float)(bf16)acc[i][j + t + 4][e], co[e], si[e], 1.f, ra, rb);
+                lo[t][e] = (bf16)ra; hi[t][e] = (bf16)rb;
+              }
+            }
+            store_pair16(crow, nb + j * 16 + fq * 4, lo[0], lo[1], fq);
+            store_pair16(crow, nb + (j + 4) * 16 + fq * 4, hi[0], hi[1], fq);
+          }
+        }
+      } else {
+#pragma unroll
+        for (int i = 0; i < MT; ++i) {
+          const int m = m0 + wm * TM + i * 16 + fr;
+          if (m >= p.M) continue;
+#pragma unroll
+          for (int j = 0; j < NT; j += 2)
+            w4_store_frag2<EPI_PLAIN>(p, acc[i][j], acc[i][j + 1], m, nb + j * 16 + fq * 4, fq);
+        }
+      }
+      return;
+    }
+  }
 #define W4_EPILOGUE(KIND)                                                                                              \
   _Pragma("unroll") for (int i = 0; i < MT; ++i) {                                                                      \
     const int m = m0 + wm * TM + i * 16 + fr;                                                                           \
@@ -911,9 +955,12 @@
   return vlb_gemm_bf16_ws(A, lda, W, ldw, C, ldc, M, N, K, bias, residual, ldr, act, A2, lda2, W2, ldw2, K2, nullptr, 0, stream);
 }
 
+struct RopeEpilogue { const float* cs; const float* sn; const int* pos; int S, cols; bool fused; };
+
 static int gemm_impl(const void* A, int lda, const void* W, int ldw, void* C, int ldc, int M, int N, int K,
                      const void* bias, const void* residual, int ldr, int act, const void* A2, int lda2,
-                     const void* W2, int ldw2, int K2, void* ws, int64_t ws_bytes, void* stream, void* aux, int ldaux);
+                     const void* W2, int ldw2, int K2, void* ws, int64_t ws_bytes, void* stream, void* aux, int ldaux,
+                     RopeEpilogue* rope = nullptr);
 
 extern "C" int vlb_gemm_bf16_ws(const void* A, int lda, const void* W, int ldw, void* C, int ldc, int M, int N, int K,
                                 const void* bias, const void* residual, int ldr, int act, const void* A2, int lda2,
@@ -930,9 +977,24 @@
                    stream, GU, ldgu);
 }
 
+extern "C" int vlb_gemm_rope_qk(const void* A, int lda, const void* W, int ldw, void* C, int ldc, int M, int N, int K,
+                                const void* A2, int lda2, const void* W2, int ldw2, int K2, const float* cos_t,
+                                const float* sin_t, const int* pos, int rope_S, int rope_cols, void* ws, int64_t ws_bytes,
+                                void* stream) {
+  VLB_REQUIRE(cos_t && sin_t && rope_S > 0 && (((uintptr_t)cos_t | (uintptr_t)sin_t) % 16) == 0,
+              "gemm_rope_qk: rope tables must be 16-byte aligned fp32 [S, 64] with S > 0");
+  VLB_REQUIRE(rope_cols > 0 && rope_cols % 128 == 0 && rope_cols <= N, "gemm_rope_qk: rope_cols=%d must be whole 128-wide heads within N", rope_cols);
+  RopeEpilogue r{cos_t, sin_t, pos, rope_S, rope_cols, false};
+  const int rc = gemm_impl(A, lda, W, ldw, C, ldc, M, N, K, nullptr, nullptr, 0, VLB_ACT_NONE, A2, lda2, W2, ldw2, K2, ws, ws_bytes,
+                           stream, nullptr, 0, &r);
+  if (rc != VLB_OK || r.fused) return rc;
+  return vlb_rope_inplace(C, ldc, cos_t, sin_t, M, rope_S, rope_cols / 128, 128, 1, pos, stream);
+}
+
 static int gemm_impl(const void* A, int lda, const void* W, int ldw, void* C, int ldc, int M, int N, int K,
                      const void* bias, const void* residual, int ldr, int act, const void* A2, int lda2,
-                     const void* W2, int ldw2, int K2, void* ws, int64_t ws_bytes, void* stream, void* aux, int ldaux) {
+                     const void* W2, int ldw2, int K2, void* ws, int64_t ws_bytes, void* stream, void* aux, int ldaux,
+                     RopeEpilogue* rope) {
   VLB_REQUIRE(A && W && C, "gemm: null operand");
   VLB_REQUIRE(!ws || ((uintptr_t)ws % 16) == 0, "gemm: workspace must be 16-byte aligned");
   const bool ws_ok = ws && ws_bytes >= vlb_gemm_workspace_bytes();
@@ -957,6 +1019,11 @@
   a.lda = lda; a.ldw = ldw; a.ldc = ldc; a.ldr = ldr; a.lda2 = lda2; a.ldw2 = ldw2;
   a.act = act; a.tiles_m = 0; a.tiles_n = 0; a.tile0 = 0; a.split_n = 1; a.grid = 0; a.drop_thresh = 0; a.drop_key = 0; a.drop_scale = 1.f;
   a.ws = nullptr; a.k_splits = 0; a.tail_tiles = 0; a.order = pick_order(M, N, K); a.aux = (bf16*)aux; a.ldaux = ldaux;
+  a.rope_cos = nullptr; a.rope_sin = nullptr; a.rope_pos = nullptr; a.rope_S = 0; a.rope_cols = 0;
+  auto with_rope = [&](GemmArgs& g) {
+    g.act = VLB_ACT_ROPE_QK; g.rope_cos = rope->cs; g.rope_sin = rope->sn; g.rope_pos = rope->pos; g.rope_S = rope->S;
+    g.rope_cols = rope->cols; rope->fused = true;
+  };
   a.wide = ((uintptr_t)C % 16) == 0 && ldc % 8 == 0 && (!aux || (((uintptr_t)aux % 16) == 0 && ldaux % 8 == 0 && (N / 2) % 8 == 0));
   hipStream_t s = as_stream(stream);
   const bool vec_ok = (ldc % 4 == 0) && (!residual || ldr % 4 == 0) && (!aux || (ldaux % 4 == 0 && (N / 2) % 4 == 0)) &&
@@ -988,6 +1055,7 @@
         hi.tiles_m = tm192; hi.tiles_n = tn; hi.tile0 = 0; hi.split_n = 1;
         const int rem192 = tiles192 % cus;
         hi.grid = p192.mode ? tiles192 - rem192 : tiles192;
+        if (rope && !p192.mode) with_rope(hi);
 #ifdef VLB_TOOLS
         if (abl192 == 1) return launch_w4<8, 1, 6>(hi, s);
         if (abl192 == 2) return launch_w4<8, 2, 6>(hi, s);
@@ -1017,6 +1085,12 @@
         GemmArgs lo = hi;
         lo.tile0 = tiles - rem; lo.ws = (float*)ws; lo.k_splits = p256.splits; lo.tail_tiles = rem;
         return launch_w4_splitk<8>(lo, s);
+      }
+      if (rope && w4 && g_force_tile == 0 && p256.mode == 0) {
+        GemmArgs hi = a;
+        hi.tiles_m = tm; hi.tiles_n = tn; hi.tile0 = 0; hi.split_n = 1; hi.grid = tiles;
+        with_rope(hi);
+        return launch_w4<8, 0, 8>(hi, s);
       }
     }
     if (g_tail_split && tiles > cus && rem != 0 && rem <= cus * 5 / 8) {
diff --git a/phantom_vlb_amd/csrc/ops.hip b/phantom_vlb_amd/csrc/ops.hip
--- a/phantom_vlb_amd/csrc/ops.hip
+++ b/phantom_vlb_amd/csrc/ops.hip
@@ -281,11 +281,7 @@
     const float* n = sn + (int64_t)s * half + ch * 8;
     float oa[8], ob[8];
 #pragma unroll
-    for (int i = 0; i < 8; ++i) {
-      const float co = c[i], si = sign * n[i];
-      oa[i] = a[i] * co - b[i] * si;
-      ob[i] = b[i] * co + a[i] * si;
-    }
+    for (int i = 0; i < 8; ++i) rope_pair(a[i], b[i], c[i], n[i], sign, oa[i], ob[i]);
     store8(p, oa); store8(p + half, ob);
   }
 }
diff --git a/phantom_vlb_amd/fullft.py b/phantom_vlb_amd/fullft.py
--- a/phantom_vlb_amd/fullft.py
+++ b/phantom_vlb_amd/fullft.py
@@ -20,6 +20,8 @@
 
 
 FUSED_QUANT = os.environ.get("VLB_FP8_FUSED_QUANT", "1") == "1"
+FUSE_ATTN_DELTA = True
+FUSE_ROPE_BWD = True
 
 
 def _up(n, m):
@@ -450,8 +452,10 @@
             self.wgrad(dx2, sv["a"], G(f"{pre}.wo"), fp8=self.fp8, dyTq=dq_[1])
             d_a = self._lin(dx2, li, "wo_t", xq=dq_[0])
             dqkv = ops.attention_bwd(sv["qkv"], qd, kd, sv["a"], d_a, sv["lse"], self.key_mask, B, S, g.heads, g.kv_heads,
-                                     g.head_dim, True, g.head_dim ** -0.5, layout=layout, delta=delta)
-            ops.rope_(dqkv, w.rope_cos, w.rope_sin, B, S, g.heads + g.kv_heads, g.head_dim, sign=-1, pos=pos)
+                                     g.head_dim, True, g.head_dim ** -0.5, layout=layout, delta=delta,
+                                     rope=(w.rope_cos, w.rope_sin, pos) if FUSE_ROPE_BWD else None, fuse_delta=FUSE_ATTN_DELTA)
+            if not FUSE_ROPE_BWD:
+                ops.rope_(dqkv, w.rope_cos, w.rope_sin, B, S, g.heads + g.kv_heads, g.head_dim, sign=-1, pos=pos)
             dq_ = self._dual(dqkv) or (None, None)
             self.wgrad(dqkv, sv["h1"], G(f"{pre}.wqkv"), fp8=self.fp8, dyTq=dq_[1])
             d_h1 = self._lin(dqkv, li, "wqkv_t", xq=dq_[0])
diff --git a/phantom_vlb_amd/lora.py b/phantom_vlb_amd/lora.py
--- a/phantom_vlb_amd/lora.py
+++ b/phantom_vlb_amd/lora.py
@@ -12,6 +12,9 @@
 BF16 = torch.bfloat16
 PAD = 64
 FUSE_SWIGLU_BWD = True
+FUSE_ATTN_DELTA = True
+FUSE_ROPE_BWD = True
+FUSE_ROPE_FWD = True
 MERGE_DB_U = True
 
 
@@ -236,6 +239,16 @@
         t = self._lora_t(x, blk, seeds, slot, p)
         return ops.gemm(x, W, residual=residual, a2=t, w2=blk["Bpad"]), t
 
+    def _adapted_qkv(self, x, W, blk, seeds, B, pos, slot=None, p=None):
+        g, w = self.g, self.w
+        if FUSE_ROPE_FWD and g.head_dim == 128:
+            t = self._lora_t(x, blk, seeds, slot, p)
+            return ops.gemm_rope_qk(x, W, w.rope_cos, w.rope_sin, g.max_len, (g.heads + g.kv_heads) * g.head_dim, pos=pos,
+                                    a2=t, w2=blk["Bpad"]), t
+        qkv, t = self._adapted(x, W, blk, seeds, slot=slot, p=p)
+        ops.rope_(qkv, w.rope_cos, w.rope_sin, B, g.max_len, g.heads + g.kv_heads, g.head_dim, pos=pos)
+        return qkv, t
+
     def _adapted_mlp_in(self, x, lw, blk, seeds, slot, p=None, save=True):
         if self.gu_il:
             t = self._lora_t(x, blk, seeds, slot, p)
@@ -266,8 +279,7 @@
             lw = backbone.layer_weights(li)
             sd = [self._seed(li, k) for k in range(7)]
             h1 = ops.rmsnorm(x, lw["in_norm"], g.rms_eps)
-            qkv, t_qkv = self._adapted(h1, lw["wqkv"], lay["qkv"], sd[0:3], slot=(li, 0))
-            ops.rope_(qkv, w.rope_cos, w.rope_sin, B, S, g.heads + g.kv_heads, g.head_dim, pos=pos)
+            qkv, t_qkv = self._adapted_qkv(h1, lw["wqkv"], lay["qkv"], sd[0:3], B, pos, slot=(li, 0))
             a, lse = ops.attention_fwd(qkv[:, :qd], qkv[:, qd:qd + kd], qkv[:, qd + kd:], B, S, g.heads, g.kv_heads,
                                        g.head_dim, True, g.head_dim ** -0.5, key_mask=key_mask, need_lse=True,
                                        layout=layout)
@@ -289,8 +301,7 @@
         for li, lay in enumerate(self.layers):
             lw = backbone.layer_weights(li)
             h = ops.rmsnorm(x, lw["in_norm"], g.rms_eps)
-            qkv, _ = self._adapted(h, lw["wqkv"], lay["qkv"], None, slot=(li, 0), p=0.0)
-            ops.rope_(qkv, w.rope_cos, w.rope_sin, B, S, g.heads + g.kv_heads, g.head_dim, pos=pos)
+            qkv, _ = self._adapted_qkv(h, lw["wqkv"], lay["qkv"], None, B, pos, slot=(li, 0), p=0.0)
             a = ops.attention_fwd(qkv[:, :qd], qkv[:, qd:qd + kd], qkv[:, qd + kd:], B, S, g.heads, g.kv_heads, g.head_dim,
                                   True, g.head_dim ** -0.5, key_mask=key_mask, layout=layout)
             x, _ = self._adapted(a, lw["wo"], lay["o"], None, residual=x, slot=(li, 1), p=0.0)
@@ -359,8 +370,10 @@
             d_a = self._group_backward(li, "o", dx2, sv["a"], sv["t_o"], sd[3:4], lw["wo_t"], True)
             qkv = sv["qkv"]
             dqkv = ops.attention_bwd(qkv, qd, kd, sv["a"], d_a, sv["lse"], self.key_mask, B, S, g.heads, g.kv_heads,
-                                     g.head_dim, True, g.head_dim ** -0.5, layout=layout, delta=delta)
-            ops.rope_(dqkv, w.rope_cos, w.rope_sin, B, S, g.heads + g.kv_heads, g.head_dim, sign=-1, pos=pos)
+                                     g.head_dim, True, g.head_dim ** -0.5, layout=layout, delta=delta,
+                                     rope=(w.rope_cos, w.rope_sin, pos) if FUSE_ROPE_BWD else None, fuse_delta=FUSE_ATTN_DELTA)
+            if not FUSE_ROPE_BWD:
+                ops.rope_(dqkv, w.rope_cos, w.rope_sin, B, S, g.heads + g.kv_heads, g.head_dim, sign=-1, pos=pos)
             need_dx = li > 0
             d_h1 = self._group_backward(li, "qkv", dqkv, sv["h1"], sv["t_qkv"], sd[0:3], lw["wqkv_t"], need_dx)
             if need_dx:
diff --git a/phantom_vlb_amd/ops.py b/phantom_vlb_amd/ops.py
--- a/phantom_vlb_amd/ops.py
+++ b/phantom_vlb_amd/ops.py
@@ -121,6 +121,26 @@
                                    _p(a2), a2.stride(0) if a2 is not None else 0, _p(w2),
                                    w2.stride(0) if w2 is not None else 0, K2, _p(ws), ws.numel() if ws is not None else 0,
                                    _stream()), "vlb_gemm_bf16")
+    return out
+
+
+def gemm_rope_qk(a, w, cos, sin, S, rope_cols, pos=None, a2=None, w2=None):
+    _dev(a)
+    M, K = a.shape
+    N = w.shape[0]
+    assert w.shape[1] == K and a.stride(1) == 1 and w.stride(1) == 1
+    assert cos.dtype == torch.float32 and sin.dtype == torch.float32 and cos.shape[1] == 64 and cos.is_contiguous() and sin.is_contiguous()
+    out = torch.empty(M, N, dtype=BF16, device=a.device)
+    K2 = 0
+    if a2 is not None:
+        K2 = a2.shape[1]
+        assert w2.shape == (N, K2) and a2.shape[0] == M
+    ws = _gemm_workspace(a.device) if K + K2 >= 4096 and M * N > 256 * 192 * 256 else None
+    with _Timed("qkv+rope", M, N, K, K2):
+        check(lib.vlb_gemm_rope_qk(a.data_ptr(), a.stride(0), w.data_ptr(), w.stride(0), out.data_ptr(), out.stride(0), M, N, K,
+                                   _p(a2), a2.stride(0) if a2 is not None else 0, _p(w2), w2.stride(0) if w2 is not None else 0,
+                                   K2, cos.data_ptr(), sin.data_ptr(), _p(pos), S, rope_cols, _p(ws),
+                                   ws.numel() if ws is not None else 0, _stream()), "vlb_gemm_rope_qk")
     return out
 
 
@@ -252,7 +272,8 @@
 
 
 def attention_bwd(qkv, qd, kd, out, dout, lse, key_mask, B, S, Hq, Hkv, D, causal, scale, layout=None, delta=None,
-                  dq_acc=None):
+                  dq_acc=None, rope=None, fuse_delta=False):
+    rope_S = S
     cu, rows = None, B * S
     if layout is not None and layout.packed:
         B, S, cu, rows = layout.B, layout.smax, layout.cu, layout.rows
@@ -263,13 +284,20 @@
         dq_acc = _attn_workspace(rows * qd, qkv.device)
     assert delta.numel() >= B * Hq * S and (dq_acc is None or dq_acc.numel() >= rows * qd)
     dqkv = torch.empty_like(qkv)
-    check(lib.vlb_attention_bwd(qkv.data_ptr(), qkv.stride(0), qkv[:, qd:].data_ptr(), qkv.stride(0),
-                                qkv[:, qd + kd:].data_ptr(), qkv.stride(0), out.data_ptr(), out.stride(0),
-                                dout.data_ptr(), dout.stride(0), lse.data_ptr(), _p(key_mask),
-                                dqkv.data_ptr(), dqkv.stride(0), dqkv[:, qd:].data_ptr(), dqkv.stride(0),
-                                dqkv[:, qd + kd:].data_ptr(), dqkv.stride(0), delta.data_ptr(), _p(dq_acc),
-                                B, S, Hq, Hkv, D, 1 if causal else 0, float(scale), _p(cu), rows, _stream()),
-          "vlb_attention_bwd")
+    args = (qkv.data_ptr(), qkv.stride(0), qkv[:, qd:].data_ptr(), qkv.stride(0),
+            qkv[:, qd + kd:].data_ptr(), qkv.stride(0), out.data_ptr(), out.stride(0),
+            dout.data_ptr(), dout.stride(0), lse.data_ptr(), _p(key_mask),
+            dqkv.data_ptr(), dqkv.stride(0), dqkv[:, qd:].data_ptr(), dqkv.stride(0),
+            dqkv[:, qd + kd:].data_ptr(), dqkv.stride(0), delta.data_ptr(), _p(dq_acc),
+            B, S, Hq, Hkv, D, 1 if causal else 0, float(scale), _p(cu), rows)
+    if rope is None and not fuse_delta:
+        check(lib.vlb_attention_bwd(*args, _stream()), "vlb_attention_bwd")
+        return dqkv
+    cos, sin, pos = rope if rope is not None else (None, None, None)
+    assert rope is None or (cos.dtype == torch.float32 and sin.dtype == torch.float32 and cos.shape[1] == D // 2
+                            and cos.is_contiguous() and sin.is_contiguous())
+    check(lib.vlb_attention_bwd_fused(*args, 1 if fuse_delta else 0, _p(cos), _p(sin), _p(pos), rope_S, _stream()),
+          "vlb_attention_bwd_fused")
     return dqkv
 
 
```

New measurement: 15.09 clips/s (median of 6 runs). No clear change (+0.5%).
